# Sue1347/SMSUT-MedicalImgSegmentation

Measured on AMD Instinct MI355X. Metric: slices/sec uganConsisTrainer step @256x256, higher is better.
Workload: dtype f32

## Files before the change

### include/smsut_hip.h

```cpp
#ifndef SMSUT_HIP_H
#define SMSUT_HIP_H

#include <stdint.h>

#ifdef __cplusplus
extern "C" {
#endif

int smsut_conv2d_fwd_generic(const float* x, const float* w, const float* bias , float* y, int N, int H,
                             int W, int Cin, int Ho, int Wo, int Cout, int KH, int KW, int stride, int pad,
                             void* stream);
int smsut_conv2d_dgrad_generic(const float* gy, const float* w, float* gx, int N, int H, int W, int Cin, int Ho, int Wo,
                               int Cout, int KH, int KW, int stride, int pad, void* stream);
int64_t smsut_conv2d_wgrad_generic_ws(int N, int Ho, int Wo, int Cin, int Cout, int KH, int KW);
int smsut_conv2d_wgrad_generic(const float* x, const float* gy, float* gw, float* workspace, int N, int H, int W,
                               int Cin, int Ho, int Wo, int Cout, int KH, int KW, int stride, int pad, void* stream);

int smsut_conv2d_mfma_supported(int KS, int stride, int pad, int Kdim, int Ndim);
int smsut_conv2d_fwd_mfma(const float* x, const float* w, float* y, int N, int H, int W, int Kdim, int Ndim, int KS,
                          int transposed, void* stream);
int smsut_conv2d_mfma_tiles(int N, int H, int W, int Kdim, int Ndim, int KS, int f16);
int smsut_conv2d_mfma_persistent(int N, int H, int W, int Kdim, int Ndim, int KS, int f16);
int smsut_conv2d_dgrad_mfma_bwdstats(const float* gy, const float* w, float* gz, float* stats, const float* y1,
                                     const float* mean, const float* rstd, const float* gamma, const float* beta,
// ... 9 lines not shown
                              int transposed, const float* wu, void* stream);
int smsut_conv2d_fwd_mfma_stats_pre(const float* x, const float* w, float* y, float* stats, int N, int H, int W, int Kdim,
                                    int Ndim, int KS, const float* wu, void* stream);
int smsut_conv2d_dgrad_mfma_bwdstats_pre(const float* gy, const float* w, float* gz, float* stats, const float* y1,
                                         const float* mean, const float* rstd, const float* gamma, const float* beta,
                                         float slope, int N, int H, int W, int Kdim, int Ndim, const float* wu, void* stream);
int smsut_conv2d_fwd_mfma_stats_inaff_pre(const float* x, const float* w, float* y, float* stats, const float* mean,
                                          const float* rstd, const float* gamma, const float* beta, float slope, int N, int H,
                                          int W, int Kdim, int Ndim, const float* wu, void* stream);
int smsut_conv2d_fwd_mfma_stats_cat_pre(const float* xa, const float* xb, const float* w, float* y, float* stats, int N, int H,
                                        int W, int Kdim, int Ndim, const float* wu, void* stream);
int smsut_conv2d_fwd_mfma_split_pre(const float* x, const float* w, float* ya, float* yb, int split, int N, int H, int W,
                                    int Kdim, int Ndim, int transposed, const float* wu, void* stream);
int smsut_conv2d_fwd_mfma_stats_sc_pre(const float* x, const float* xb, const float* w, const float* wsc, float* y, float* ysc,
                                       float* stats, float* stats_sc, int N, int H, int W, int Kdim, int Ndim, const float* wu,
                                       void* stream);
int smsut_conv2d_wgrad_mfma_supported(int KS, int stride, int pad, int Cin, int Cout);
int64_t smsut_conv2d_wgrad_mfma_ws(int N, int H, int W, int Cin, int Cout, int KS);
int smsut_conv2d_wgrad_mfma(const float* x, const float* gy, float* gw, float* workspace, int N, int H, int W, int Cin,
                            int Cout, int KS, void* stream);

int smsut_conv1x1_supported(int Kdim, int Ndim);
int smsut_conv1x1_tiles(int N, int HW, int Ndim);
int smsut_conv1x1_fwd(const float* x, const float* w, float* y, float* stats , int N, int HW, int Kdim,
                      int Ndim, int transposed, void* stream);
int64_t smsut_conv1x1_wgrad_ws(int N, int HW, int Cin, int Cout);
int smsut_conv1x1_wgrad(const float* x, const float* gy, float* gw, float* workspace, int N, int HW, int Cin, int Cout,
                        void* stream);

int smsut_conv2d_fwd_mfma_stats_inaff(const float* x, const float* w, float* y, float* stats, const float* mean,
                                      const float* rstd, const float* gamma, const float* beta, float slope, int N, int H,
                                      int W, int Kdim, int Ndim, void* stream);
int smsut_conv2d_wgrad_mfma_inaff(const float* x, const float* gy, float* gw, float* workspace, const float* mean,
                                  const float* rstd, const float* gamma, const float* beta, float slope, int N, int H, int W,
                                  int Cin, int Cout, void* stream);
int smsut_conv2d_wgrad_mfma_slabs(const float* x, const float* gy, float* workspace, const float* mean, const float* rstd,
                                  const float* gamma, const float* beta, float slope, int N, int H, int W, int Cin, int Cout,
                                  void* stream);
int smsut_conv2d_mfma_form(int N, int H, int W, int Kdim, int Ndim, int sc_dgrad);

int smsut_conv2d_mfma_cat_supported(int N, int H, int W, int Kdim, int Ndim);
int smsut_conv2d_fwd_mfma_stats_cat(const float* xa, const float* xb, const float* w, float* y, float* stats, int N, int H,
                                    int W, int Kdim, int Ndim, void* stream);
int smsut_conv2d_fwd_sc_supported(int N, int H, int W, int Kdim, int Ndim, int cat);
int smsut_conv2d_fwd_mfma_stats_sc(const float* x, const float* xb , const float* w, const float* wsc, float* y,
                                   float* ysc, float* stats, float* stats_sc, int N, int H, int W, int Kdim, int Ndim,
                                   void* stream);
int smsut_conv2d_fwd_sc_f16_supported(int N, int H, int W, int Kdim, int Ndim, int cat);
int smsut_conv2d_fwd_mfma_stats_sc_f16(const float* x, const float* xb, const float* w, const float* wsc, float* y, float* ysc,
                                       float* stats, float* stats_sc, int N, int H, int W, int Kdim, int Ndim, void* stream);
int smsut_conv2d_dgrad_sc_supported(int N, int H, int W, int Cout, int Cin, int split);
int smsut_conv2d_dgrad_mfma_sc(const float* gy, const float* gs, const float* w, const float* wsc, float* gxa,
                               float* gxb , int split, int N, int H, int W, int Cout, int Cin, void* stream);
int smsut_conv2d_wgrad_sc_supported(int N, int H, int W, int Cin, int Cout);
int64_t smsut_conv2d_wgrad_sc_ws(int N, int H, int W, int Cin, int Cout);
int smsut_conv2d_wgrad_mfma_sc(const float* xa, const float* xb , int ca, const float* gy, const float* gs,
                               float* gw10, float* workspace, int N, int H, int W, int Cin, int Cout, void* stream);
int smsut_conv2d_wgrad_mfma_cat(const float* xa, const float* xb, int ca, const float* gy, float* gw, float* workspace,
                                int N, int H, int W, int Cin, int Cout, int KS, void* stream);
int smsut_conv2d_fwd_mfma_stats_sc_fin(const float* x, const float* xb , const float* w, const float* wsc, float* y,
                                       float* ysc, float* stats, float* stats_sc, int* tickets, float* mean, float* rstd,
                                       float* mean_sc, float* rstd_sc, float eps, int N, int H, int W, int Kdim, int Ndim,
                                       const float* wu , void* stream);
int smsut_conv2d_fwd_mfma_stats_inaff_fin(const float* x, const float* w, float* y, float* stats, const float* mean,
                                          const float* rstd, const float* gamma, const float* beta, float slope, int* tickets,
                                          float* mean_out, float* rstd_out, float eps, int N, int H, int W, int Kdim, int Ndim,
                                          const float* wu , void* stream);
int smsut_conv2d_dgrad_mfma_bwdstats_fin(const float* gy, const float* w, float* gz, float* stats, const float* y1,
                                         const float* mean, const float* rstd, const float* gamma, const float* beta, float slope,
                                         int* tickets, float* a_mean, float* b_mean, int N, int H, int W, int Kdim, int Ndim,
                                         const float* wu , void* stream);
int smsut_conv2d_wgrad_pair_supported(int NA, int NB, int H, int W, int Cin, int Cout, int cat, int aff, int sc);
int64_t smsut_conv2d_wgrad_pair_ws(int NA, int NB, int H, int W, int Cin, int Cout, int cat, int aff, int sc);
int smsut_conv2d_wgrad_pair(const float* xA, const float* x2A , const float* gyA, const float* gsA ,
                            const float* meanA , const float* rstdA , int NA, const float* xB,
                            const float* x2B , const float* gyB, const float* gsB ,
                            const float* meanB , const float* rstdB , int NB, int ca,
                            const float* gamma , const float* beta , float slope, float* gw, float* workspace,
                            int H, int W, int Cin, int Cout, void* stream);
int smsut_conv2d_wgrad_pair_slabs(const float* xA, const float* gyA, const float* meanA , const float* rstdA ,
                                  int NA, const float* xB, const float* gyB, const float* meanB ,
                                  const float* rstdB , int NB, const float* gamma , const float* beta ,
                                  float slope, float* workspace, int H, int W, int Cin, int Cout, void* stream);
int smsut_conv1x1_fwd_cat(const float* xa, const float* xb, int ca, const float* w, float* y, float* stats ,
                          int N, int HW, int Kdim, int Ndim, void* stream);
int smsut_conv1x1_wgrad_cat(const float* xa, const float* xb, int ca, const float* gy, float* gw, float* workspace, int N,
                            int HW, int Cin, int Cout, void* stream);

int smsut_conv2d_mfma_split_supported(int N, int H, int W, int Kdim, int Ndim, int split);
int smsut_conv2d_fwd_mfma_split(const float* x, const float* w, float* ya, float* yb, int split, int N, int H, int W,
                                int Kdim, int Ndim, int transposed, void* stream);
int smsut_conv1x1_fwd_split(const float* x, const float* w, float* ya, float* yb, int split, int N, int HW, int Kdim,
                            int Ndim, int transposed, void* stream);

int smsut_conv2d_f16_supported(int KS, int Kdim, int Ndim);
int smsut_conv2d_fwd_mfma_f16(const float* x, const float* w, float* y, const float* gsc , int N, int H, int W,
                              int Kdim, int Ndim, int KS, int transposed, void* stream);
int smsut_conv2d_fwd_mfma_stats_f16(const float* x, const float* w, float* y, float* stats, int N, int H, int W, int Kdim,
                                    int Ndim, int KS, void* stream);
int smsut_conv2d_fwd_mfma_stats_cat_f16(const float* xa, const float* xb, const float* w, float* y, float* stats, int N, int H,
                                        int W, int Kdim, int Ndim, void* stream);
int smsut_conv2d_fwd_mfma_split_f16(const float* x, const float* w, float* ya, float* yb, const float* gsc ,
                                    int split, int N, int H, int W, int Kdim, int Ndim, int transposed, void* stream);
int smsut_conv2d_f16_hs_supported(int N, int H, int W, int Kdim, int Ndim, int cat);
int smsut_conv2d_fwd_mfma_stats_f16_hs(const float* x, const float* xb , const float* w, void* y16, float* stats, int N,
                                       int H, int W, int Kdim, int Ndim, void* stream);
int smsut_conv2d_fwd_mfma_stats_f16_hsx(const void* x16, const float* w, void* y16, float* stats, int N, int H, int W, int Kdim,
                                        int Ndim, void* stream);
int smsut_conv2d_fwd_mfma_stats_inaff_f16_hsx(const void* y1_16, const float* w, void* y16, float* stats, const float* mean,
                                              const float* rstd, const float* gamma, const float* beta, float slope, int N, int H,
                                              int W, int Kdim, int Ndim, void* stream);
int smsut_conv2d_fwd_mfma_stats_sc_f16_hs(const float* x, const float* xb , const float* w, const float* wsc, void* y16,
                                          void* ysc16, float* stats, float* stats_sc, int N, int H, int W, int Kdim, int Ndim,
                                          void* stream);
int smsut_conv2d_dgrad_mfma_bwdstats_f16_hs(const float* gy, const float* w, float* gz, float* stats, const void* y1_16,
                                            const float* mean, const float* rstd, const float* gamma, const float* beta,
                                            const float* gsc , float slope, int N, int H, int W, int Kdim, int Ndim,
                                            void* stream);
int smsut_conv2d_dgrad_sc_f16_supported(int N, int H, int W, int Cout, int Cin, int split);
int smsut_conv2d_dgrad_mfma_sc_f16(const float* gy, const float* gs, const float* w, const float* wsc, float* gxa,
                                   float* gxb , const float* gsc, int split, int N, int H, int W, int Cout, int Cin,
                                   void* stream);
int smsut_conv2d_dgrad_mfma_bwdstats_f16(const float* gy, const float* w, float* gz, float* stats, const float* y1,
                                         const float* mean, const float* rstd, const float* gamma, const float* beta,
                                         const float* gsc , float slope, int N, int H, int W, int Kdim, int Ndim,
                                         void* stream);
int smsut_conv2d_wgrad_f16_supported(int N, int H, int W, int Cin, int Cout);
int64_t smsut_conv2d_wgrad_f16_ws(int N, int H, int W, int Cin, int Cout);
int smsut_conv2d_wgrad_f16(const float* x, const float* x2 , int ca, const float* gy, float* gw, float* workspace,
                           const float* gsc , int N, int H, int W, int Cin, int Cout, void* stream);
int smsut_conv2d_wgrad_f16_xh(const void* x16, const float* gy, float* gw, float* workspace, const float* gsc , int N,
                              int H, int W, int Cin, int Cout, void* stream);
int smsut_conv2d_wgrad_f16_xh_inaff(const void* y1_16, const float* gy, float* gw, float* workspace, const float* gsc ,
                                    const float* mean, const float* rstd, const float* gamma, const float* beta, float slope, int N,
                                    int H, int W, int Cin, int Cout, void* stream);
int smsut_conv2d_wgrad_sc_f16_supported(int N, int H, int W, int Cin, int Cout);
int64_t smsut_conv2d_wgrad_sc_f16_ws(int N, int H, int W, int Cin, int Cout);
int smsut_conv2d_wgrad_sc_f16(const float* x, const float* x2 , int ca, const float* gy, const float* gs, float* gw10,
                              float* workspace, const float* gsc, int N, int H, int W, int Cin, int Cout, void* stream);
int64_t smsut_absmax_scale_ws(int64_t n);
int smsut_absmax_scale(const float* x, int64_t n, float* out2, float* workspace, void* stream);
int smsut_absmax_scale2(const float* x, int64_t n, const float* x2, int64_t n2, float* out2, float* workspace, void* stream);
int smsut_absmax_finish(const float* amax, int n, float* out2, void* stream);

int smsut_conv2d_k4_supported(int Cin, int Cout);
int smsut_conv2d_k4_fwd(const float* x, const float* w, float* y, int N, int H, int W, int Cin, int Cout, int transposed,
                        void* stream);
int64_t smsut_conv2d_k4_wgrad_ws(int N, int H, int W, int Cin, int Cout);
int smsut_conv2d_k4_wgrad(const float* x, const float* gy, float* gw, float* workspace, int N, int H, int W, int Cin, int Cout,
                          void* stream);

int smsut_conv1x1_thin_supported(int Cin, int Cout);
int smsut_conv1x1_thin_dgrad(const float* gy, const float* w, float* gx, int N, int HW, int Cin, int Cout, void* stream);
int64_t smsut_conv1x1_thin_wgrad_ws(int Cin);
int smsut_conv1x1_thin_wgrad(const float* x, const float* gy, float* gw, float* workspace, int N, int HW, int Cin,
                             int Cout, void* stream);

int smsut_conv2d_small_supported(int KS, int Cin, int Cout);
int smsut_conv2d_small_fwd(const float* x, const float* w, const float* bias , float* y, int N, int H, int W,
                           int Cin, int Ho, int Wo, int Cout, int KS, int stride, int pad, void* stream);
int smsut_conv2d_small_dgrad(const float* gy, const float* w, float* gx, int N, int H, int W, int Cin, int Ho, int Wo,
                             int Cout, int KS, int stride, int pad, void* stream);
int smsut_conv2d_flat_wgrad_supported(int KS, int stride, int Cin, int Cout);
int64_t smsut_conv2d_flat_wgrad_ws(int N, int Ho, int Wo, int Cin, int Cout, int KS);
int smsut_conv2d_flat_wgrad(const float* x, const float* gy, float* gw, float* workspace, int N, int H, int W, int Cin,
                            int Ho, int Wo, int Cout, int KS, int stride, int pad, void* stream);
// ... 248 lines not shown
```

### smsut-medicalimgsegmentation_amd/csrc/conv1x1.hip

```cpp
#include "common.h"

namespace {

typedef float f32x4 __attribute__((ext_vector_type(4)));
constexpr int TPB = 256;

__device__ __forceinline__ f32x4 mfma16(float a, float b, f32x4 c) {
  return __builtin_amdgcn_mfma_f32_16x16x4f32(a, b, c, 0, 0, 0);
}

template <int MR, int NR, bool DUAL = false, bool PS = false>
__global__ void __launch_bounds__(TPB)
conv1x1_fwd(const float* __restrict__ x, const float* __restrict__ w, float* __restrict__ y, float* __restrict__ stats,
            int64_t P, int HW, int Kdim, int Ndim, int transposed, float* __restrict__ y2 = nullptr, int split = 0,
            const float* __restrict__ x2 = nullptr, int ca = 0, int ps_w = 0) {
  constexpr int CO_T = 16 * NR;
  extern __shared__ float w_s[];
  const int tid = threadIdx.x, lane = tid & 63, wave = tid >> 6;
  const int lm = lane & 15, kq = lane >> 4;
  const int co0 = blockIdx.y * CO_T;
  const int chunks = (Kdim + 15) / 16;
  for (int u = tid; u < chunks * 4 * CO_T; u += TPB) {
    const int n = u % CO_T;
    const int kg = (u / CO_T) * 4;
    const int ng = co0 + n;
    float4 v = make_float4(0.f, 0.f, 0.f, 0.f);
    if (ng < Ndim && kg < Kdim) {
      if constexpr (PS) {
        const int cout = Ndim >> 2, tap = ng / cout;
        const float* p = w + ((size_t)tap * Kdim + kg) * cout + (ng - tap * cout);
        v.x = p[0]; v.y = p[cout]; v.z = p[2 * (size_t)cout]; v.w = p[3 * (size_t)cout];
      } else if (!transposed) {
        const float* p = w + (size_t)kg * Ndim + ng;
        v.x = p[0]; v.y = p[Ndim]; v.z = p[2 * (size_t)Ndim]; v.w = p[3 * (size_t)Ndim];
      } else {
        v = *(const float4*)(w + (size_t)ng * Kdim + kg);
      }
    }
    *(float4*)(w_s + (size_t)u * 4) = v;
  }
  __syncthreads();

  const int64_t p0 = ((int64_t)blockIdx.x * 4 + wave) * (16 * MR);
  if (p0 >= P) return;
  f32x4 acc[MR][NR];
#pragma unroll
  for (int i = 0; i < MR; ++i)
#pragma unroll
    for (int j = 0; j < NR; ++j) acc[i][j] = (f32x4){0.f, 0.f, 0.f, 0.f};
  const float* xp[MR];
  const float* xq[MR];
  bool pok[MR];
  const int sa = DUAL ? ca : Kdim;
#pragma unroll
  for (int i = 0; i < MR; ++i) {
    const int64_t p = p0 + i * 16 + lm;
    pok[i] = p < P;
    xp[i] = x + (size_t)(pok[i] ? p : 0) * sa + 4 * kq;
    xq[i] = DUAL ? x2 + (size_t)(pok[i] ? p : 0) * (Kdim - ca) + 4 * kq - ca : xp[i];
  }
  for (int c = 0; c < chunks; ++c) {
    const bool kok = c * 16 + 4 * kq < Kdim;
    const bool second = DUAL && c * 16 >= ca;
    f32x4 a[MR], b[NR];
#pragma unroll
    for (int i = 0; i < MR; ++i)
      a[i] = (pok[i] && kok) ? *(const f32x4*)((second ? xq[i] : xp[i]) + c * 16) : (f32x4){0.f, 0.f, 0.f, 0.f};
#pragma unroll
    for (int j = 0; j < NR; ++j) b[j] = *(const f32x4*)(w_s + ((size_t)(c * 4 + kq) * CO_T + j * 16 + lm) * 4);
#pragma unroll
    for (int s = 0; s < 4; ++s)
#pragma unroll
      for (int i = 0; i < MR; ++i)
#pragma unroll
        for (int j = 0; j < NR; ++j) acc[i][j] = mfma16(a[i][s], b[j][s], acc[i][j]);
  }
#pragma unroll
  for (int j = 0; j < NR; ++j) {
    const int co = co0 + j * 16 + lm;
    const bool hi = y2 && co0 + j * 16 >= split;
    float* const yo = hi ? y2 : y;
    const int os = !y2 ? Ndim : (hi ? Ndim - split : split);
    const int oc = hi ? co - split : co;
// ... 56 lines not shown
#pragma unroll
  for (int i = 0; i < CIT; ++i)
#pragma unroll
    for (int j = 0; j < COT; ++j) acc[i][j] = (f32x4){0.f, 0.f, 0.f, 0.f};
  bool iok[CIT], jok[COT];
#pragma unroll
  for (int i = 0; i < CIT; ++i) iok[i] = ci0 + i * 16 + lm < Cin;
#pragma unroll
  for (int j = 0; j < COT; ++j) jok[j] = co0 + j * 16 + lm < Cout;
  CatSrc xs[CIT];
#pragma unroll
  for (int i = 0; i < CIT; ++i) xs[i] = cat_src(x, x2, Cin, ca, ci0 + i * 16);
  const float* gb = gy + co0 + lm;
  [[maybe_unused]] const int cout = Cout >> 2;
  [[maybe_unused]] int ps_tap[COT], ps_cc[COT];
  if constexpr (PS) {
#pragma unroll
    for (int j = 0; j < COT; ++j) { ps_tap[j] = (co0 + j * 16) / cout; ps_cc[j] = co0 + j * 16 - ps_tap[j] * cout + lm; }
  }
  constexpr int UNR = W1_UNR;
  for (int64_t p0 = pb + 4 * wave + kq; p0 - kq < pe; p0 += 16 * UNR) {
    float a[UNR][CIT], b[UNR][COT];
#pragma unroll
    for (int u = 0; u < UNR; ++u) {
      const int64_t p = p0 + 16 * u;
      const bool ok = p < pe;
#pragma unroll
      for (int i = 0; i < CIT; ++i) a[u][i] = (ok && iok[i]) ? xs[i].p[(size_t)p * xs[i].stride + ci0 + i * 16 + lm - xs[i].coff] : 0.f;
      if constexpr (PS) {
        const int row = (int)p / ps_w;
        const int wx = (int)p - row * ps_w;
#pragma unroll
        for (int j = 0; j < COT; ++j)
          b[u][j] = (ok && jok[j]) ? gy[((size_t)(2 * row + (ps_tap[j] >> 1)) * (2 * ps_w) + 2 * wx + (ps_tap[j] & 1)) * cout + ps_cc[j]] : 0.f;
      } else {
#pragma unroll
        for (int j = 0; j < COT; ++j) b[u][j] = (ok && jok[j]) ? gb[(size_t)p * Cout + j * 16] : 0.f;
      }
    }
#pragma unroll
    for (int u = 0; u < UNR; ++u)
#pragma unroll
      for (int i = 0; i < CIT; ++i)
#pragma unroll
        for (int j = 0; j < COT; ++j) acc[i][j] = mfma16(a[u][i], b[u][j], acc[i][j]);
  }
  for (int src = 1; src < 4; ++src) {
    __syncthreads();
    if (wave == src) {
#pragma unroll
      for (int i = 0; i < CIT; ++i)
#pragma unroll
        for (int j = 0; j < COT; ++j) *(f32x4*)(red + ((size_t)(i * COT + j) * 64 + lane) * 4) = acc[i][j];
    }
    __syncthreads();
    if (wave == 0) {
#pragma unroll
      for (int i = 0; i < CIT; ++i)
#pragma unroll
        for (int j = 0; j < COT; ++j) acc[i][j] += *(const f32x4*)(red + ((size_t)(i * COT + j) * 64 + lane) * 4);
    }
  }
  if (wave == 0) {
    float* out = part + (size_t)blockIdx.x * Cin * Cout;
#pragma unroll
    for (int i = 0; i < CIT; ++i)
#pragma unroll
      for (int j = 0; j < COT; ++j) {
        const int co = co0 + j * 16 + lm;
#pragma unroll
        for (int r = 0; r < 4; ++r) {
          const int ci = ci0 + i * 16 + 4 * kq + r;
          if constexpr (PS) {
            if (ci < Cin && co < Cout) out[((size_t)ps_tap[j] * Cin + ci) * cout + ps_cc[j]] = acc[i][j][r];
          } else if (ci < Cin && co < Cout) out[(size_t)ci * Cout + co] = acc[i][j][r];
        }
      }
  }
}

__global__ void __launch_bounds__(TPB)
sum_parts(const float* __restrict__ part, float* __restrict__ out, int wsize, int splits) {
  __shared__ float4 sm[TPB];
  const int col = threadIdx.x & 15, sl = threadIdx.x >> 4;
  const int e = (blockIdx.x * 16 + col) * 4;
  float4 t0 = make_float4(0.f, 0.f, 0.f, 0.f), t1 = t0, t2 = t0, t3 = t0;
  if (e < wsize) {
    int c = sl;
    for (; c + 48 < splits; c += 64) {
      const float4 v0 = *(const float4*)(part + (size_t)c * wsize + e);
      const float4 v1 = *(const float4*)(part + (size_t)(c + 16) * wsize + e);
      const float4 v2 = *(const float4*)(part + (size_t)(c + 32) * wsize + e);
      const float4 v3 = *(const float4*)(part + (size_t)(c + 48) * wsize + e);
      t0.x += v0.x; t0.y += v0.y; t0.z += v0.z; t0.w += v0.w; t1.x += v1.x; t1.y += v1.y; t1.z += v1.z; t1.w += v1.w;
      t2.x += v2.x; t2.y += v2.y; t2.z += v2.z; t2.w += v2.w; t3.x += v3.x; t3.y += v3.y; t3.z += v3.z; t3.w += v3.w;
    }
    for (; c < splits; c += 16) {
      const float4 v = *(const float4*)(part + (size_t)c * wsize + e);
      t0.x += v.x; t0.y += v.y; t0.z += v.z; t0.w += v.w;
    }
  }
  sm[threadIdx.x] = make_float4((t0.x + t1.x) + (t2.x + t3.x), (t0.y + t1.y) + (t2.y + t3.y), (t0.z + t1.z) + (t2.z + t3.z),
                                (t0.w + t1.w) + (t2.w + t3.w));
  __syncthreads();
  if (sl == 0 && e < wsize) {
    float4 t = sm[col];
    for (int l = 1; l < 16; ++l) { const float4 v = sm[l * 16 + col]; t.x += v.x; t.y += v.y; t.z += v.z; t.w += v.w; }
    *(float4*)(out + e) = t;
  }
}

struct Plan1 { int splits; int64_t pps; };
inline Plan1 plan_wgrad1(int64_t P, int Cin, int Cout, int cit, int cot) {
  const int slabs = ((Cin + 16 * cit - 1) / (16 * cit)) * ((Cout + 16 * cot - 1) / (16 * cot));
  int64_t want = (1024 + slabs - 1) / slabs;
  const int64_t maxs = P / 256 > 0 ? P / 256 : 1;
  if (want > maxs) want = maxs;
  if (want < 1) want = 1;
  Plan1 p;
  p.pps = ((P + want - 1) / want + 15) / 16 * 16;
  p.splits = (int)((P + p.pps - 1) / p.pps);
  return p;
}


constexpr int THIN_MAX = 8;

template <int CI>
__global__ void __launch_bounds__(TPB)
thin1x1_dgrad(const float* __restrict__ gy, const float* __restrict__ w, float* __restrict__ gx, int64_t P, int CO) {
  constexpr int Q = CI / 4;
  __shared__ float wt[THIN_MAX * CI];
  for (int u = threadIdx.x; u < THIN_MAX * CI; u += TPB) {
    const int k = u / CI, ci = u % CI;
    wt[u] = k < CO ? w[ci * CO + k] : 0.f;
  }
  __syncthreads();
  const int64_t total = P * Q;
  for (int64_t i = (int64_t)blockIdx.x * TPB + threadIdx.x; i < total; i += (int64_t)gridDim.x * TPB) {
    const int c4 = (int)(i % Q);
    const int64_t px = i / Q;
    float g[THIN_MAX];
#pragma unroll
    for (int k = 0; k < THIN_MAX; ++k) g[k] = k < CO ? gy[px * CO + k] : 0.f;
    f32x4 o = {0.f, 0.f, 0.f, 0.f};
#pragma unroll
    for (int k = 0; k < THIN_MAX; ++k) o += g[k] * *(const f32x4*)(wt + k * CI + c4 * 4);
    *(f32x4*)(gx + i * 4) = o;
  }
}

template <int CI>
__global__ void __launch_bounds__(TPB)
thin1x1_wgrad(const float* __restrict__ x, const float* __restrict__ gy, float* __restrict__ part, int64_t P, int CO) {
  constexpr int Q = CI / 4;
  static_assert(Q <= 64 && (Q & (Q - 1)) == 0, "lanes sharing a channel group sit Q apart inside a wave");
  __shared__ float sm[4 * Q * 4 * THIN_MAX];
  f32x4 acc[THIN_MAX];
#pragma unroll
  for (int k = 0; k < THIN_MAX; ++k) acc[k] = (f32x4){0.f, 0.f, 0.f, 0.f};
  const int64_t total = P * Q;
  const int64_t stride = (int64_t)gridDim.x * TPB;
  auto step = [&](int64_t i) {
    const int64_t px = i / Q;
    const f32x4 xv = *(const f32x4*)(x + i * 4);
#pragma unroll
    for (int k = 0; k < THIN_MAX; ++k) {
      const float g = k < CO ? gy[px * CO + k] : 0.f;
      acc[k] += g * xv;
    }
  };
  int64_t i = (int64_t)blockIdx.x * TPB + threadIdx.x;
  for (; i + stride < total; i += 2 * stride) { step(i); step(i + stride); }
  for (; i < total; i += stride) step(i);
  for (int off = Q; off < 64; off <<= 1) {
#pragma unroll
    for (int k = 0; k < THIN_MAX; ++k)
#pragma unroll
      for (int j = 0; j < 4; ++j) acc[k][j] += __shfl_xor(acc[k][j], off, 64);
  }
  const int lane = threadIdx.x & 63, wv = threadIdx.x >> 6;
  if (lane < Q) {
#pragma unroll
    for (int k = 0; k < THIN_MAX; ++k) *(f32x4*)(sm + ((wv * Q + lane) * THIN_MAX + k) * 4) = acc[k];
  }
  __syncthreads();
  if (threadIdx.x < Q) {
    const int c4 = threadIdx.x;
#pragma unroll
    for (int k = 0; k < THIN_MAX; ++k) {
      f32x4 t = *(const f32x4*)(sm + ((0 * Q + c4) * THIN_MAX + k) * 4);
#pragma unroll
// ... 44 lines not shown
  SMSUT_REQUIRE(!x2 || (!transposed && ca > 0 && ca < Kdim && ca % 16 == 0 && (Kdim - ca) % 4 == 0));
  const int64_t P = (int64_t)N * HW;
  const int mr = (P / 256 >= 512) ? 4 : 1;
  SMSUT_REQUIRE(!stats || HW % (16 * mr) == 0);
  const int nr = Ndim <= 16 ? 1 : 2;
  const int chunks = (Kdim + 15) / 16;
  const size_t sh = (size_t)chunks * 4 * 16 * nr * 4 * sizeof(float);
  dim3 grid((unsigned)cdiv64(P, 64 * mr), (Ndim + 16 * nr - 1) / (16 * nr));
  hipStream_t st = (hipStream_t)stream;
#define LAUNCH1X1(M, R)                                                                                                      \
  do {                                                                                                                       \
    if (x2) conv1x1_fwd<M, R, true><<<grid, TPB, sh, st>>>(x, w, y, stats, P, HW, Kdim, Ndim, transposed, y2, split, x2, ca); \
    else conv1x1_fwd<M, R, false><<<grid, TPB, sh, st>>>(x, w, y, stats, P, HW, Kdim, Ndim, transposed, y2, split, nullptr, 0); \
  } while (0)
  if (mr == 4 && nr == 2) LAUNCH1X1(4, 2);
  else if (mr == 4) LAUNCH1X1(4, 1);
  else if (nr == 2) LAUNCH1X1(1, 2);
  else LAUNCH1X1(1, 1);
#undef LAUNCH1X1
  SMSUT_LAUNCH_CHECK();
  return SMSUT_OK;
}

int smsut_conv1x1_fwd(const float* x, const float* w, float* y, float* stats, int N, int HW, int Kdim, int Ndim,
                      int transposed, void* stream) {
  return conv1x1_fwd_launch(x, w, y, stats, N, HW, Kdim, Ndim, transposed, stream, nullptr, 0);
}

int smsut_conv1x1_fwd_cat(const float* xa, const float* xb, int ca, const float* w, float* y, float* stats, int N, int HW,
                          int Kdim, int Ndim, void* stream) {
  SMSUT_REQUIRE(xb);
  return conv1x1_fwd_launch(xa, w, y, stats, N, HW, Kdim, Ndim, 0, stream, nullptr, 0, xb, ca);
}

int smsut_conv1x1_fwd_split(const float* x, const float* w, float* ya, float* yb, int split, int N, int HW, int Kdim,
                            int Ndim, int transposed, void* stream) {
  SMSUT_REQUIRE(yb);
  return conv1x1_fwd_launch(x, w, ya, nullptr, N, HW, Kdim, Ndim, transposed, stream, yb, split);
}

int smsut_convT2x2_ps_supported(int Cin, int Cout) {
  return Cout == 16 && Cin <= 256 && smsut_conv1x1_supported(Cin, 4 * Cout);
}

int smsut_convT2x2_fwd_ps(const float* x, const float* w, float* y, int N, int H, int W, int Cin, int Cout, void* stream) {
  SMSUT_REQUIRE(x && w && y && N > 0 && H > 0 && W > 0 && smsut_convT2x2_ps_supported(Cin, Cout));
  const int64_t P = (int64_t)N * H * W;
  SMSUT_REQUIRE(P * 4 * Cout < (1ll << 31));
  const int Nd = 4 * Cout;
  const int mr = (P / 256 >= 512) ? 4 : 1;
  const int nr = (Nd % 64 == 0) ? 4 : 2;
  const int chunks = (Cin + 15) / 16;
  const size_t sh = (size_t)chunks * 4 * 16 * nr * 4 * sizeof(float);
  dim3 grid((unsigned)cdiv64(P, 64 * mr), Nd / (16 * nr));
  hipStream_t st = (hipStream_t)stream;
#define PS_GO(M, R) conv1x1_fwd<M, R, false, true><<<grid, TPB, sh, st>>>(x, w, y, nullptr, P, H * W, Cin, Nd, 0, nullptr, 0, nullptr, 0, W)
  if (mr == 4 && nr == 4) PS_GO(4, 4);
  else if (mr == 4) PS_GO(4, 2);
  else if (nr == 4) PS_GO(1, 4);
  else PS_GO(1, 2);
#undef PS_GO
  SMSUT_LAUNCH_CHECK();
  return SMSUT_OK;
}

int64_t smsut_convT2x2_wgrad_ps_ws(int N, int H, int W, int Cin, int Cout) {
  const int cit = Cin > 16 ? 2 : 1;
  return (int64_t)plan_wgrad1((int64_t)N * H * W, Cin, 4 * Cout, cit, 2).splits * Cin * 4 * Cout;
}

int smsut_convT2x2_wgrad_ps(const float* x, const float* gy, float* gw, float* workspace, int N, int H, int W, int Cin,
                            int Cout, void* stream) {
  SMSUT_REQUIRE(x && gy && gw && workspace && N > 0 && H > 0 && W > 0 && smsut_convT2x2_ps_supported(Cin, Cout));
  const int64_t P = (int64_t)N * H * W;
  SMSUT_REQUIRE(P * 4 * Cout < (1ll << 31));
  const int Nd = 4 * Cout;
  const int cit = Cin > 16 ? 2 : 1;
  const Plan1 p = plan_wgrad1(P, Cin, Nd, cit, 2);
  dim3 grid(p.splits, (Cin + 16 * cit - 1) / (16 * cit), Nd / 32);
  hipStream_t st = (hipStream_t)stream;
  if (cit == 2) conv1x1_wgrad<2, 2, true><<<grid, TPB, 0, st>>>(x, gy, workspace, P, Cin, Nd, p.pps, nullptr, 0, W);
  else conv1x1_wgrad<1, 2, true><<<grid, TPB, 0, st>>>(x, gy, workspace, P, Cin, Nd, p.pps, nullptr, 0, W);
  const int wsize = Cin * Nd;
  sum_parts<<<(wsize + 63) / 64, TPB, 0, st>>>(workspace, gw, wsize, p.splits);
  SMSUT_LAUNCH_CHECK();
  return SMSUT_OK;
}

int64_t smsut_conv1x1_wgrad_ws(int N, int HW, int Cin, int Cout) {
  const int cit = Cin > 16 ? 2 : 1, cot = Cout > 16 ? 2 : 1;
  return (int64_t)plan_wgrad1((int64_t)N * HW, Cin, Cout, cit, cot).splits * Cin * Cout;
}

static int conv1x1_wgrad_launch(const float* x, const float* gy, float* gw, float* workspace, int N, int HW, int Cin,
                                int Cout, void* stream, const float* x2, int ca) {
  SMSUT_REQUIRE(x && gy && gw && workspace && N > 0 && HW > 0 && Cin > 0 && Cout > 0);
  SMSUT_REQUIRE(!x2 || (ca > 0 && ca < Cin && ca % 16 == 0));
  SMSUT_REQUIRE(((int64_t)Cin * Cout) % 4 == 0);
  const int64_t P = (int64_t)N * HW;
  const int cit = Cin > 16 ? 2 : 1, cot = Cout > 16 ? 2 : 1;
  const Plan1 p = plan_wgrad1(P, Cin, Cout, cit, cot);
  dim3 grid(p.splits, (Cin + 16 * cit - 1) / (16 * cit), (Cout + 16 * cot - 1) / (16 * cot));
  hipStream_t st = (hipStream_t)stream;
  if (cit == 2 && cot == 2) conv1x1_wgrad<2, 2><<<grid, TPB, 0, st>>>(x, gy, workspace, P, Cin, Cout, p.pps, x2, ca);
  else if (cit == 2) conv1x1_wgrad<2, 1><<<grid, TPB, 0, st>>>(x, gy, workspace, P, Cin, Cout, p.pps, x2, ca);
  else if (cot == 2) conv1x1_wgrad<1, 2><<<grid, TPB, 0, st>>>(x, gy, workspace, P, Cin, Cout, p.pps, x2, ca);
  else conv1x1_wgrad<1, 1><<<grid, TPB, 0, st>>>(x, gy, workspace, P, Cin, Cout, p.pps, x2, ca);
  const int wsize = Cin * Cout;
  sum_parts<<<(wsize + 63) / 64, TPB, 0, st>>>(workspace, gw, wsize, p.splits);
  SMSUT_LAUNCH_CHECK();
  return SMSUT_OK;
}

int smsut_conv1x1_wgrad(const float* x, const float* gy, float* gw, float* workspace, int N, int HW, int Cin, int Cout,
                        void* stream) {
  return conv1x1_wgrad_launch(x, gy, gw, workspace, N, HW, Cin, Cout, stream, nullptr, 0);
}

int smsut_conv1x1_wgrad_cat(const float* xa, const float* xb, int ca, const float* gy, float* gw, float* workspace, int N,
                            int HW, int Cin, int Cout, void* stream) {
  SMSUT_REQUIRE(xb);
  return conv1x1_wgrad_launch(xa, gy, gw, workspace, N, HW, Cin, Cout, stream, xb, ca);
}

int smsut_conv1x1_thin_supported(int Cin, int Cout) {
  return (Cin == 8 || Cin == 16 || Cin == 32 || Cin == 64) && Cout >= 1 && Cout <= THIN_MAX;
}

int smsut_conv1x1_thin_dgrad(const float* gy, const float* w, float* gx, int N, int HW, int Cin, int Cout, void* stream) {
  SMSUT_REQUIRE(gy && w && gx && N > 0 && HW > 0 && smsut_conv1x1_thin_supported(Cin, Cout));
  const int64_t P = (int64_t)N * HW;
  hipStream_t st = (hipStream_t)stream;
  const int grid = ew_grid(P * (Cin / 4));
  switch (Cin) {
    case 8: thin1x1_dgrad<8><<<grid, TPB, 0, st>>>(gy, w, gx, P, Cout); break;
    case 16: thin1x1_dgrad<16><<<grid, TPB, 0, st>>>(gy, w, gx, P, Cout); break;
    case 32: thin1x1_dgrad<32><<<grid, TPB, 0, st>>>(gy, w, gx, P, Cout); break;
    default: thin1x1_dgrad<64><<<grid, TPB, 0, st>>>(gy, w, gx, P, Cout); break;
  }
  SMSUT_LAUNCH_CHECK();
  return SMSUT_OK;
}

int64_t smsut_conv1x1_thin_wgrad_ws(int Cin) { return (int64_t)THIN_WGRAD_BLOCKS * Cin * THIN_MAX; }

int smsut_conv1x1_thin_wgrad(const float* x, const float* gy, float* gw, float* workspace, int N, int HW, int Cin,
                             int Cout, void* stream) {
  SMSUT_REQUIRE(x && gy && gw && workspace && N > 0 && HW > 0 && smsut_conv1x1_thin_supported(Cin, Cout));
  const int64_t P = (int64_t)N * HW;
  hipStream_t st = (hipStream_t)stream;
  int blocks = (int)cdiv64(P * (Cin / 4), 2 * TPB);
  if (blocks > THIN_WGRAD_BLOCKS) blocks = THIN_WGRAD_BLOCKS;
  switch (Cin) {
    case 8: thin1x1_wgrad<8><<<blocks, TPB, 0, st>>>(x, gy, workspace, P, Cout); break;
    case 16: thin1x1_wgrad<16><<<blocks, TPB, 0, st>>>(x, gy, workspace, P, Cout); break;
    case 32: thin1x1_wgrad<32><<<blocks, TPB, 0, st>>>(x, gy, workspace, P, Cout); break;
    default: thin1x1_wgrad<64><<<blocks, TPB, 0, st>>>(x, gy, workspace, P, Cout); break;
  }
  thin1x1_wsum<<<(Cin * THIN_MAX / 4 + 3) / 4, TPB, 0, st>>>(workspace, gw, blocks, Cin, Cout);
  SMSUT_LAUNCH_CHECK();
  return SMSUT_OK;
}

}
```

### smsut-medicalimgsegmentation_amd/csrc/conv_mfma_wgrad.hip

```cpp
#include "conv_mfma.h"
#include "conv_wgrad_rr.h"

namespace {

typedef short s16x4 __attribute__((ext_vector_type(4)));
__device__ __forceinline__ f32x4 mfmak(h4 a, h4 b, f32x4 c) { return mfma16h(a, b, c); }
__device__ __forceinline__ f32x4 mfmak(h8 a, h8 b, f32x4 c) { return mfma32h(a, b, c); }

constexpr int WTH = 8;
#ifndef WG_RR_UNROLL
#define WG_RR_UNROLL 2
#endif
#ifndef WG_KS_UNROLL
#define WG_KS_UNROLL 4
#endif
#ifndef WG11_MIN_BLOCKS
#define WG11_MIN_BLOCKS 1
#endif
#ifndef WTS_STRIDE_VALUE
#define WTS_STRIDE_VALUE 36
#endif
constexpr int WTS_STRIDE_SC = 68;
constexpr int WTS_STRIDE = WTS_STRIDE_VALUE;

template <int KS, int CIT, int COT, bool DUAL = false, bool INAFF = false, bool C8 = false, bool SC8 = false>
__global__ void __launch_bounds__(TPB, (KS == 3 && CIT == 1 && COT == 1 && !INAFF) ? WG11_MIN_BLOCKS : 1)
conv_mfma_wgrad(const float* __restrict__ x, const float* __restrict__ gy, float* __restrict__ part, int N, int H,
                int W, int Cin, int Cout, int tiles_x, int tiles_y, int tiles_per_split, int gsc, int nci,
                const float* __restrict__ x2 = nullptr, int ca = 0, AffRef aff = AffRef{},
                const float* __restrict__ gs = nullptr) {
  static_assert(!SC8 || C8, "fused shortcut weight gradient of the 8-channel form");
  static_assert(!C8 || (KS == 3 && CIT == 1 && !DUAL && !INAFF), "8-channel form: plain 3x3");
  constexpr int KK = KS * KS;
  constexpr int PAD = (KS - 1) / 2;
  constexpr int IH = WTH + KS - 1, IW = TW + KS - 1;
  constexpr int CI_T = 16 * CIT, CO_T = 16 * COT;
  constexpr int SI = (CI_T % 32 == 16) ? CI_T : CI_T + 16;
  constexpr int SO = (CO_T % 32 == 16) ? CO_T : CO_T + 16;
  constexpr int NG = C8 ? (KK + 1) / 2 : KK;
  constexpr int NACC = (NG + (SC8 ? 1 : 0)) * CIT * COT;
  extern __shared__ float smem[];
  float* in_s = smem;
  float* gy_s = smem + IH * IW * SI;
  [[maybe_unused]] float* gs_s = gy_s + WTH * TW * SO;

  const int tid = threadIdx.x;
  const int lane = tid & 63, wave = tid >> 6;
  const int lm = lane & 15, kq = lane >> 4;
  const int split = blockIdx.x;
  const int tg = blockIdx.y / nci;
  const int ci0 = (blockIdx.y % nci) * CI_T, co0 = blockIdx.z * CO_T;
  const int Wg = W * gsc;
  const int tiles_img = tiles_x * tiles_y;
  const int total_tiles = N * tiles_img;
  const int t_begin = split * tiles_per_split;
  const int t_end = min(t_begin + tiles_per_split, total_tiles);

  f32x4 acc[NACC];
#pragma unroll
  for (int i = 0; i < NACC; ++i) acc[i] = (f32x4){0.f, 0.f, 0.f, 0.f};

  constexpr int NIN = (IH * IW * (CI_T / 4) + TPB - 1) / TPB;
  constexpr int NGY = (WTH * TW * (CO_T / 4) + TPB - 1) / TPB;
  float4 rin[NIN], rgy[NGY];
  [[maybe_unused]] float4 rgs[NGY];
  int in_yx[NIN], in_c[NIN], in_lds[NIN], gy_yx[NGY], gy_c[NGY], gy_lds[NGY];
#pragma unroll
  for (int i = 0; i < NIN; ++i) {
    const int u = tid + i * TPB;
    const int q = u % (CI_T / 4), pix = u / (CI_T / 4);
    const int c = ci0 + 4 * q;
    in_yx[i] = (u < IH * IW * (CI_T / 4) && c < Cin) ? (((pix / IW) << 8) | (pix % IW)) : -1;
    in_c[i] = c;
    in_lds[i] = pix * SI + 4 * q;
  }
#pragma unroll
  for (int i = 0; i < NGY; ++i) {
    const int u = tid + i * TPB;
    const int q = u % (CO_T / 4), pix = u / (CO_T / 4);
    const int c = co0 + 4 * q;
    gy_yx[i] = (u < WTH * TW * (CO_T / 4) && c < Cout) ? (((pix / TW) << 8) | (pix % TW)) : -1;
    gy_c[i] = c;
    gy_lds[i] = pix * SO + 4 * q;
  }
// ... 486 lines not shown
        for (int k = 0; k < 9; ++k) {
          const int ti = (wave + 4 * k) >> 1;
          const int tap = ti >> 1, i = ti & 1;
          const auto a = tr_rows(x_h + (i * NPX + (r + tap / KS) * IW + tap % KS) * 16, IW * 16);
          acc[k] = mfmak(a, b, acc[k]);
        }
        if constexpr (SC) {
          const auto bs = tr_rows(s_h + (jt * NPG + r * TW) * 16, TW * 16);
          const auto a = tr_rows(x_h + ((wave >> 1) * NPX + (r + 1) * IW + 1) * 16, IW * 16);
          acc[9] = mfmak(a, bs, acc[9]);
        }
      }
    } else {
#pragma unroll
      for (int rr = 0; rr < WTH / 4; rr += RS) {
        const int r = wave * (WTH / 4) + rr;
        decltype(tr_rows(g_h, 0)) b[COT];
#pragma unroll
        for (int j = 0; j < COT; ++j) b[j] = tr_rows(g_h + (j * NPG + r * TW) * 16, TW * 16);
#pragma unroll
        for (int tap = 0; tap < KK; ++tap)
#pragma unroll
          for (int i = 0; i < CIT; ++i) {
            const auto a = tr_rows(x_h + (i * NPX + (r + tap / KS) * IW + tap % KS) * 16, IW * 16);
#pragma unroll
            for (int j = 0; j < COT; ++j) acc[(tap * CIT + i) * COT + j] = mfmak(a, b[j], acc[(tap * CIT + i) * COT + j]);
          }
        if constexpr (SC) {
          decltype(tr_rows(s_h, 0)) bs[COT];
#pragma unroll
          for (int j = 0; j < COT; ++j) bs[j] = tr_rows(s_h + (j * NPG + r * TW) * 16, TW * 16);
#pragma unroll
          for (int i = 0; i < CIT; ++i) {
            const auto a = tr_rows(x_h + (i * NPX + (r + 1) * IW + 1) * 16, IW * 16);
#pragma unroll
            for (int j = 0; j < COT; ++j) acc[(9 * CIT + i) * COT + j] = mfmak(a, bs[j], acc[(9 * CIT + i) * COT + j]);
          }
        }
      }
    }
  }
  if constexpr (TS) {
    const int jt = wave & 1;
    float* out = part + (size_t)split * KR * Cin * Cout + (size_t)(ci0 + 4 * kq) * Cout + co0 + jt * 16 + lm;
#pragma unroll
    for (int k = 0; k < KR; ++k) {
      const int ti = (wave + 4 * k) >> 1;
      float* o = out + ((ti >> 1) * Cin + (ti & 1) * 16) * Cout;
#pragma unroll
      for (int r = 0; r < 4; ++r) o[r * Cout] = acc[k][r] * gi;
    }
  } else {
    float* red = smem;
    for (int src = 1; src < 4; ++src) {
      __syncthreads();
      if (wave == src) {
#pragma unroll
        for (int k = 0; k < NACC; ++k) *(f32x4*)(red + ((size_t)k * 64 + lane) * 4) = acc[k];
      }
      __syncthreads();
      if (wave == 0) {
#pragma unroll
        for (int k = 0; k < NACC; ++k) acc[k] += *(const f32x4*)(red + ((size_t)k * 64 + lane) * 4);
      }
    }
    if (wave == 0) {
      float* out = part + (size_t)split * KR * Cin * Cout;
#pragma unroll
      for (int tap = 0; tap < KR; ++tap)
#pragma unroll
        for (int i = 0; i < CIT; ++i)
#pragma unroll
          for (int j = 0; j < COT; ++j)
#pragma unroll
            for (int r = 0; r < 4; ++r)
              out[((size_t)tap * Cin + ci0 + i * 16 + 4 * kq + r) * Cout + co0 + j * 16 + lm] = acc[(tap * CIT + i) * COT + j][r] * gi;
    }
  }
}

template <int COLS>
__global__ void __launch_bounds__(TPB)
sum_splits(const float* __restrict__ part, float* __restrict__ out, int wsize, int splits) {
  constexpr int LANES = TPB / COLS;
  __shared__ float4 sm[TPB];
  const int col = threadIdx.x % COLS, sl = threadIdx.x / COLS;
  const int e = (blockIdx.x * COLS + col) * 4;
  float4 t0 = make_float4(0.f, 0.f, 0.f, 0.f), t1 = t0, t2 = t0, t3 = t0;
  if (e < wsize) {
    const float* p = part + e;
    int c = sl;
    for (; c + 3 * LANES < splits; c += 4 * LANES) {
      const float4 v0 = *(const float4*)(p + (size_t)c * wsize);
      const float4 v1 = *(const float4*)(p + (size_t)(c + LANES) * wsize);
      const float4 v2 = *(const float4*)(p + (size_t)(c + 2 * LANES) * wsize);
      const float4 v3 = *(const float4*)(p + (size_t)(c + 3 * LANES) * wsize);
      t0.x += v0.x; t0.y += v0.y; t0.z += v0.z; t0.w += v0.w;
      t1.x += v1.x; t1.y += v1.y; t1.z += v1.z; t1.w += v1.w;
      t2.x += v2.x; t2.y += v2.y; t2.z += v2.z; t2.w += v2.w;
      t3.x += v3.x; t3.y += v3.y; t3.z += v3.z; t3.w += v3.w;
    }
    for (; c < splits; c += LANES) {
      const float4 v = *(const float4*)(p + (size_t)c * wsize);
      t0.x += v.x; t0.y += v.y; t0.z += v.z; t0.w += v.w;
    }
  }
  sm[threadIdx.x] = make_float4((t0.x + t1.x) + (t2.x + t3.x), (t0.y + t1.y) + (t2.y + t3.y),
                                (t0.z + t1.z) + (t2.z + t3.z), (t0.w + t1.w) + (t2.w + t3.w));
  __syncthreads();
  if (sl == 0 && e < wsize) {
    float4 t = sm[col];
    for (int l = 1; l < LANES; ++l) {
      const float4 v = sm[l * COLS + col];
      t.x += v.x; t.y += v.y; t.z += v.z; t.w += v.w;
    }
    *(float4*)(out + e) = t;
  }
}

inline void launch_sum_splits(const float* part, float* out, int wsize, int splits, hipStream_t st) {
  if (wsize >= 32768) sum_splits<64><<<(wsize + 255) / 256, TPB, 0, st>>>(part, out, wsize, splits);
  else if (wsize >= 8192) sum_splits<32><<<(wsize + 127) / 128, TPB, 0, st>>>(part, out, wsize, splits);
  else sum_splits<16><<<(wsize + 63) / 64, TPB, 0, st>>>(part, out, wsize, splits);
}

constexpr int PW_UNR = 8;
__global__ void __launch_bounds__(TPB)
plane_wgrad(const float* __restrict__ x, const float* __restrict__ gy, float* __restrict__ gw, int N, int H, int W, int Cin,
            int Cout, const float* __restrict__ x2 = nullptr, int ca = 0) {
  __shared__ float red[3 * 4 * 64 * 4];
  const int lane = threadIdx.x & 63, wave = threadIdx.x >> 6;
  const int lm = lane & 15, kq = lane >> 4;
  const int ci0 = blockIdx.x * 32, co0 = blockIdx.y * 32;
  const int tap = blockIdx.z, dy = tap / 3 - 1, dx = tap % 3 - 1;
  const int HW = H * W, P = N * HW;
  f32x4 acc[2][2];
#pragma unroll
  for (int i = 0; i < 2; ++i)
#pragma unroll
    for (int j = 0; j < 2; ++j) acc[i][j] = (f32x4){0.f, 0.f, 0.f, 0.f};
  const CatSrc s0 = cat_src(x, x2, Cin, ca, ci0), s1 = cat_src(x, x2, Cin, ca, ci0 + 16);
  const float* xa0 = s0.p + ci0 + lm - s0.coff;
  const float* xa1 = s1.p + ci0 + 16 + lm - s1.coff;
  const float* gb = gy + co0 + lm;
  constexpr int BLK = 4 * PW_UNR;
  for (int p0 = wave * BLK; p0 < P; p0 += 4 * BLK) {
    const int pk = p0 + kq;
    int cn = pk / HW;
    const int r = pk - cn * HW;
    int cy = r / W, cx = r - cy * W;
    float a[PW_UNR][2], b[PW_UNR][2];
#pragma unroll
    for (int u = 0; u < PW_UNR; ++u) {
      const int p = p0 + 4 * u + kq;
      const int yy = cy + dy, xx = cx + dx;
      const bool ok = p < P;
      const bool in = ok && yy >= 0 && yy < H && xx >= 0 && xx < W;
      const size_t pix = (size_t)((cn * H + yy) * W + xx);
      const float* gp = gb + (size_t)p * Cout;
      a[u][0] = in ? xa0[pix * s0.stride] : 0.f; a[u][1] = in ? xa1[pix * s1.stride] : 0.f;
      b[u][0] = ok ? gp[0] : 0.f; b[u][1] = ok ? gp[16] : 0.f;
      cx += 4;
      if (cx >= W) { cx -= W; if (++cy == H) { cy = 0; ++cn; } }
    }
#pragma unroll
    for (int u = 0; u < PW_UNR; ++u)
#pragma unroll
      for (int i = 0; i < 2; ++i)
#pragma unroll
        for (int j = 0; j < 2; ++j) acc[i][j] = mfma16(a[u][i], b[u][j], acc[i][j]);
  }
  if (wave > 0) {
#pragma unroll
    for (int t = 0; t < 4; ++t) *(f32x4*)(red + (((wave - 1) * 4 + t) * 64 + lane) * 4) = acc[t >> 1][t & 1];
  }
  __syncthreads();
  if (wave == 0) {
#pragma unroll
    for (int t = 0; t < 4; ++t) {
      f32x4 v = acc[t >> 1][t & 1];
#pragma unroll
      for (int w4 = 0; w4 < 3; ++w4) v += *(const f32x4*)(red + ((w4 * 4 + t) * 64 + lane) * 4);
      float* o = gw + ((size_t)tap * Cin + ci0 + (t >> 1) * 16 + 4 * kq) * Cout + co0 + (t & 1) * 16 + lm;
#pragma unroll
      for (int r = 0; r < 4; ++r) o[(size_t)r * Cout] = v[r];
    }
  }
}

template <int COT>
__global__ void __launch_bounds__(TPB)
conv_k4_wgrad(const float* __restrict__ x, const float* __restrict__ gy, float* __restrict__ part, int N, int Hi, int Wi,
              int Ho, int Wo, int Cin, int Cout, int tiles_x, int tiles_y, int tiles_per_split) {
  constexpr int KS = 4, KK = 16, PAD = 1;
  constexpr int IH = WTH + KS - 1, IW = TW + KS - 1;
  constexpr int CO_T = 16 * COT, SI = 16, SO = (CO_T % 32 == 16) ? CO_T : CO_T + 16;
  constexpr int NACC = KK * COT;
  extern __shared__ float smem[];
  float* in_s = smem;
  float* gy_s = smem + IH * IW * SI;
  const int tid = threadIdx.x, lane = tid & 63, wave = tid >> 6;
  const int lm = lane & 15, kq = lane >> 4;
  const int split = blockIdx.x, ci0 = blockIdx.y * 16, co0 = blockIdx.z * CO_T;
  const int tiles_img = tiles_x * tiles_y, total_tiles = N * tiles_img;
  const int t_begin = split * tiles_per_split, t_end = min(t_begin + tiles_per_split, total_tiles);
  f32x4 acc[NACC];
#pragma unroll
// ... 226 lines not shown
  }
  if (c.aff) return c.x2 ? -1 : go(conv_mfma_wgrad_ts<false, true>, sh);
  return c.x2 ? go(conv_mfma_wgrad_ts<true>, sh) : go(conv_mfma_wgrad_ts<false>, sh);
}

inline WgradCall wgrad_call(const void* x, const float* x2, int ca, const float* gy, float* part, int N, int H, int W, int Cin, int Cout,
                            void* stream) {
  WgradCall c;
  c.x = x; c.x2 = x2; c.ca = x2 ? ca : 0; c.gy = gy; c.part = part;
  c.N = N; c.H = H; c.W = W; c.Cin = Cin; c.Cout = Cout; c.stream = (hipStream_t)stream;
  return c;
}
inline int wgrad_reduce(int rc, const WgradCall& c, const WgradPlan& p, float* gw) {
  SMSUT_REQUIRE(rc == 0);
  launch_sum_splits(c.part, gw, p.rows * c.Cin * c.Cout, p.splits, c.stream);
  SMSUT_LAUNCH_CHECK();
  return SMSUT_OK;
}

int wgrad_run(const WgradCall& c, float* gw) {
  SMSUT_REQUIRE(c.x && c.gy && c.part && c.N > 0 && c.H > 0 && c.W > 0);
  SMSUT_REQUIRE(!c.x2 || (c.ca > 0 && c.ca < c.Cin && c.ca % 16 == 0 && (c.Cin - c.ca) % 4 == 0));
  const WgradKey k = c.key();
  WgradPlan p = wgrad_select(k, c.KS);
  if (p.fam == WF_RR && smsut_wgrad_rr_launch(c) != 0) p = wgrad_select(k, c.KS, true);
  if (c.b || !gw) SMSUT_REQUIRE(p.fam == WF_RR);
  if (!gw) return hipGetLastError() == hipSuccess ? p.splits : SMSUT_EINVAL;
  switch (p.fam) {
    case WF_NONE: return SMSUT_EINVAL;
    case WF_RR: return wgrad_reduce(0, c, p, gw);
    case WF_TS: return wgrad_reduce(launch_wgrad_ts(c, p), c, p, gw);
    case WF_PLANE:
      plane_wgrad<<<dim3(c.Cin / 32, c.Cout / 32, 9), TPB, 0, c.stream>>>((const float*)c.x, c.gy, gw, c.N, c.H, c.W, c.Cin, c.Cout,
                                                                        c.x2, c.ca);
      SMSUT_LAUNCH_CHECK();
      return SMSUT_OK;
    default: return wgrad_reduce(launch_wgrad_rows(c, p), c, p, gw);
  }
}

inline bool wgrad_f16_shape_ok(int N, int H, int W, int Cin, int Cout) {
  return N > 0 && H > 0 && W > 0 && H % WTH == 0 && W % TW == 0 && Cin % 16 == 0 && Cout % 16 == 0 &&
         (int64_t)N * H * W * (Cin > Cout ? Cin : Cout) < (1ll << 31);
}
WgradPlan plan_wgrad_f16(int N, int H, int W, int Cin, int Cout, bool sc) {
  WgradPlan p = plan_wgrad(N, H, W, Cin, Cout);
  p.cit = (Cin % 32 == 0) ? 2 : 1;
  p.cot = (Cout % 32 == 0) ? 2 : 1;
  p.rows = sc ? 10 : 9;
  return p;
}
template <int CI, int CO>
int launch_wgrad_f16(const WgradCall& c, const WgradPlan& p) {
  constexpr int NPX = (WTH + 2) * (TW + 2), NPG = WTH * TW;
  const bool sc = c.gs != nullptr;
  const size_t stage = (size_t)((CI * NPX + (sc ? 2 : 1) * CO * NPG) * 16 + 8) * sizeof(_Float16);
  const size_t red = (CI == 2 && CO == 2) ? 0 : (size_t)p.rows * CI * CO * 64 * 4 * sizeof(float);
  const dim3 grid(p.splits, c.Cin / (16 * CI), c.Cout / (16 * CO));
  auto go = [&](auto kern) {
    kern<<<grid, TPB, stage > red ? stage : red, c.stream>>>((const float*)c.x, c.gy, c.part, c.N, c.H, c.W, c.Cin, c.Cout, p.tiles_x,
                                                             p.tiles_y, p.tiles_per_split, c.x2, c.ca, c.gsc, c.gs,
                                                             c.aff ? *c.aff : AffRef{});
    return 0;
  };
  if (c.x_f16) {
    if (c.x2 || sc) return -1;
    return c.aff ? go(conv_f16_wgrad<CI, CO, false, false, true, true>) : go(conv_f16_wgrad<CI, CO, false, false, true>);
  }
  if (c.aff) return -1;
  if (sc) return c.x2 ? go(conv_f16_wgrad<CI, CO, true, true>) : go(conv_f16_wgrad<CI, CO, false, true>);
  return c.x2 ? go(conv_f16_wgrad<CI, CO, true, false>) : go(conv_f16_wgrad<CI, CO, false, false>);
}
int wgrad_f16_run(const WgradCall& c, float* gw) {
  SMSUT_REQUIRE(c.x && c.gy && gw && c.part && wgrad_f16_shape_ok(c.N, c.H, c.W, c.Cin, c.Cout));
  SMSUT_REQUIRE(!c.x2 || (c.ca > 0 && c.ca < c.Cin && c.ca % 16 == 0));
  const WgradPlan p = plan_wgrad_f16(c.N, c.H, c.W, c.Cin, c.Cout, c.gs != nullptr);
  const int rc = p.cit == 2 ? (p.cot == 2 ? launch_wgrad_f16<2, 2>(c, p) : launch_wgrad_f16<2, 1>(c, p))
                            : (p.cot == 2 ? launch_wgrad_f16<1, 2>(c, p) : launch_wgrad_f16<1, 1>(c, p));
  return wgrad_reduce(rc, c, p, gw);
}

}

extern "C" {

#ifdef SMSUT_STAMPS
int smsut_dbg_wgrad_stamps(void* buf, int base) {
  (void)hipMemcpyToSymbol(HIP_SYMBOL(g_stamp_base), &base, sizeof(base));
  return (int)hipMemcpyToSymbol(HIP_SYMBOL(g_stamps), &buf, sizeof(buf));
}
#endif
#ifdef SMSUT_DBG_SUM
int smsut_dbg_sum_splits(const float* part, float* out, int wsize, int splits, void* stream) {
  launch_sum_splits(part, out, wsize, splits, (hipStream_t)stream);
  return 0;
}
#endif

int smsut_conv2d_wgrad_mfma_supported(int KS, int stride, int pad, int Cin, int Cout) {
  return (KS == 1 || KS == 3) && stride == 1 && pad == (KS - 1) / 2 && wgrad_channels_ok(Cin, Cout);
}

int64_t smsut_conv2d_wgrad_mfma_ws(int N, int H, int W, int Cin, int Cout, int KS) {
  return wgrad_ws_floats(WgradKey{N, H, W, Cin, Cout, false, false, false}, KS);
}

int smsut_conv2d_wgrad_mfma(const float* x, const float* gy, float* gw, float* workspace, int N, int H, int W, int Cin,
                            int Cout, int KS, void* stream) {
  SMSUT_REQUIRE(gw);
  WgradCall c = wgrad_call(x, nullptr, 0, gy, workspace, N, H, W, Cin, Cout, stream);
  c.KS = KS;
  return wgrad_run(c, gw);
}

int smsut_conv2d_wgrad_mfma_inaff(const float* x, const float* gy, float* gw, float* workspace, const float* mean,
                                  const float* rstd, const float* gamma, const float* beta, float slope, int N, int H, int W,
                                  int Cin, int Cout, void* stream) {
  SMSUT_REQUIRE(gw && mean && rstd && gamma && beta);
  const AffRef a{mean, rstd, gamma, beta, slope};
  WgradCall c = wgrad_call(x, nullptr, 0, gy, workspace, N, H, W, Cin, Cout, stream);
  c.aff = &a;
  return wgrad_run(c, gw);
}

int smsut_conv2d_wgrad_mfma_slabs(const float* x, const float* gy, float* workspace, const float* mean, const float* rstd,
                                  const float* gamma, const float* beta, float slope, int N, int H, int W, int Cin, int Cout,
                                  void* stream) {
  SMSUT_REQUIRE(!mean || (rstd && gamma && beta));
  const AffRef a{mean, rstd, gamma, beta, slope};
  WgradCall c = wgrad_call(x, nullptr, 0, gy, workspace, N, H, W, Cin, Cout, stream);
  c.aff = mean ? &a : nullptr;
  return wgrad_run(c, nullptr);
}

int smsut_conv2d_wgrad_sc_supported(int N, int H, int W, int Cin, int Cout) {
  return wgrad_select(WgradKey{N, H, W, Cin, Cout, false, false, true}, 3).fam != WF_NONE;
}
int64_t smsut_conv2d_wgrad_sc_ws(int N, int H, int W, int Cin, int Cout) {
  return wgrad_ws_floats(WgradKey{N, H, W, Cin, Cout, false, false, true}, 3);
}
int smsut_conv2d_wgrad_mfma_sc(const float* xa, const float* xb, int ca, const float* gy, const float* gs, float* gw10,
                               float* workspace, int N, int H, int W, int Cin, int Cout, void* stream) {
  SMSUT_REQUIRE(gw10 && gs);
  WgradCall c = wgrad_call(xa, xb, ca, gy, workspace, N, H, W, Cin, Cout, stream);
  c.gs = gs;
  return wgrad_run(c, gw10);
}

int smsut_conv2d_wgrad_mfma_cat(const float* xa, const float* xb, int ca, const float* gy, float* gw, float* workspace,
                                int N, int H, int W, int Cin, int Cout, int KS, void* stream) {
  SMSUT_REQUIRE(gw && xb);
  WgradCall c = wgrad_call(xa, xb, ca, gy, workspace, N, H, W, Cin, Cout, stream);
  c.KS = KS;
  return wgrad_run(c, gw);
}

int smsut_conv2d_wgrad_pair_supported(int NA, int NB, int H, int W, int Cin, int Cout, int cat, int aff, int sc) {
  return NA > 0 && NB > 0 && wgrad_select(WgradKey{NA + NB, H, W, Cin, Cout, cat != 0, aff != 0, sc != 0}, 3).fam == WF_RR;
}
int64_t smsut_conv2d_wgrad_pair_ws(int NA, int NB, int H, int W, int Cin, int Cout, int cat, int aff, int sc) {
  return (int64_t)smsut_wgrad_rr_splits(WgradKey{NA + NB, H, W, Cin, Cout, cat != 0, aff != 0, sc != 0}) * (sc ? 10 : 9) * Cin * Cout;
}
static int wgrad_pair_run(const WgradSetB& sa, const WgradSetB& sb, int ca, const float* gamma, const float* beta, float slope, float* gw,
                          float* workspace, int H, int W, int Cin, int Cout, void* stream) {
  const bool aff = sa.mean != nullptr;
  SMSUT_REQUIRE(aff == (sa.rstd != nullptr) && (!aff || (gamma && beta)));
  const AffRef a{sa.mean, sa.rstd, gamma, beta, slope};
// ... 118 lines not shown
```

### smsut-medicalimgsegmentation_amd/csrc/conv_naive.hip

```cpp
#include "common.h"

namespace {

constexpr int TPB = 256;

struct ConvGeom {
  int N, H, W, Cin, Ho, Wo, Cout, KH, KW, stride, pad;
};

__global__ void __launch_bounds__(TPB)
conv_fwd_naive(const float* __restrict__ x, const float* __restrict__ w, const float* __restrict__ bias,
               float* __restrict__ y, ConvGeom g, int64_t total) {
  for (int64_t i = (int64_t)blockIdx.x * TPB + threadIdx.x; i < total; i += (int64_t)gridDim.x * TPB) {
    const int co = (int)(i % g.Cout);
    int64_t p = i / g.Cout;
    const int wo = (int)(p % g.Wo); p /= g.Wo;
    const int ho = (int)(p % g.Ho);
    const int n = (int)(p / g.Ho);
    float acc = bias ? bias[co] : 0.f;
    for (int kh = 0; kh < g.KH; ++kh) {
      const int hi = ho * g.stride - g.pad + kh;
      if (hi < 0 || hi >= g.H) continue;
      for (int kw = 0; kw < g.KW; ++kw) {
        const int wi = wo * g.stride - g.pad + kw;
        if (wi < 0 || wi >= g.W) continue;
        const float* xp = x + (((size_t)n * g.H + hi) * g.W + wi) * g.Cin;
        const float* wp = w + ((size_t)(kh * g.KW + kw) * g.Cin) * g.Cout + co;
        for (int ci = 0; ci < g.Cin; ++ci) acc = fmaf(xp[ci], wp[(size_t)ci * g.Cout], acc);
      }
    }
    y[i] = acc;
  }
}

__global__ void __launch_bounds__(TPB)
conv_full_window(const float* __restrict__ x, const float* __restrict__ w, const float* __restrict__ bias,
                 float* __restrict__ y, int K, int Cout) {
  __shared__ float sm4[4];
  const int n = blockIdx.x;
  for (int co = 0; co < Cout; ++co) {
    float acc = 0.f;
    for (int k = threadIdx.x; k < K; k += TPB) acc = fmaf(x[(size_t)n * K + k], w[(size_t)k * Cout + co], acc);
    const float t = block_sum_256(acc, sm4);
    if (threadIdx.x == 0) y[(size_t)n * Cout + co] = t + (bias ? bias[co] : 0.f);
  }
}

__global__ void __launch_bounds__(TPB)
conv_dgrad_naive(const float* __restrict__ gy, const float* __restrict__ w, float* __restrict__ gx, ConvGeom g,
                 int64_t total) {
  for (int64_t i = (int64_t)blockIdx.x * TPB + threadIdx.x; i < total; i += (int64_t)gridDim.x * TPB) {
    const int ci = (int)(i % g.Cin);
    int64_t p = i / g.Cin;
    const int wi = (int)(p % g.W); p /= g.W;
    const int hi = (int)(p % g.H);
    const int n = (int)(p / g.H);
    float acc = 0.f;
    for (int kh = 0; kh < g.KH; ++kh) {
      const int hn = hi + g.pad - kh;
      if (hn < 0 || hn % g.stride) continue;
      const int ho = hn / g.stride;
      if (ho >= g.Ho) continue;
      for (int kw = 0; kw < g.KW; ++kw) {
        const int wn = wi + g.pad - kw;
        if (wn < 0 || wn % g.stride) continue;
        const int wo = wn / g.stride;
        if (wo >= g.Wo) continue;
        const float* gp = gy + (((size_t)n * g.Ho + ho) * g.Wo + wo) * g.Cout;
        const float* wp = w + ((size_t)(kh * g.KW + kw) * g.Cin + ci) * g.Cout;
        int co = 0;
        if ((g.Cout & 3) == 0) {
          for (; co < g.Cout; co += 4) {
            const float4 a = *(const float4*)(gp + co);
            const float4 b = *(const float4*)(wp + co);
            acc = fmaf(a.x, b.x, acc); acc = fmaf(a.y, b.y, acc);
            acc = fmaf(a.z, b.z, acc); acc = fmaf(a.w, b.w, acc);
          }
        } else {
          for (; co < g.Cout; ++co) acc = fmaf(gp[co], wp[co], acc);
        }
      }
    }
    gx[i] = acc;
  }
}

__global__ void __launch_bounds__(TPB)
conv_wgrad_partial(const float* __restrict__ x, const float* __restrict__ gy, float* __restrict__ part, ConvGeom g,
                   int wsize, int64_t npix, int pix_per_chunk) {
  const int e = blockIdx.x * TPB + threadIdx.x;
  const int chunk = blockIdx.y;
  if (e >= wsize) return;
  const int co = e % g.Cout;
  int t = e / g.Cout;
  const int ci = t % g.Cin; t /= g.Cin;
  const int kw = t % g.KW;
  const int kh = t / g.KW;
  const int64_t p0 = (int64_t)chunk * pix_per_chunk;
  const int64_t p1 = min(p0 + (int64_t)pix_per_chunk, npix);
  int wo = (int)(p0 % g.Wo);
  const int64_t q0 = p0 / g.Wo;
  int ho = (int)(q0 % g.Ho);
  int n = (int)(q0 / g.Ho);
  float acc = 0.f;
  const float* gp = gy + (size_t)p0 * g.Cout + co;
  for (int64_t p = p0; p < p1; ++p, gp += g.Cout) {
    const int hi = ho * g.stride - g.pad + kh;
    const int wi = wo * g.stride - g.pad + kw;
    if (hi >= 0 && hi < g.H && wi >= 0 && wi < g.W)
      acc = fmaf(x[(((size_t)n * g.H + hi) * g.W + wi) * g.Cin + ci], *gp, acc);
    if (++wo == g.Wo) { wo = 0; if (++ho == g.Ho) { ho = 0; ++n; } }
  }
  part[(size_t)chunk * wsize + e] = acc;
}

__global__ void __launch_bounds__(TPB)
reduce_chunks(const float* __restrict__ part, float* __restrict__ out, int wsize, int chunks) {
  __shared__ double sm[TPB];
  const int e = blockIdx.x * 64 + (threadIdx.x & 63);
  const int lane_c = threadIdx.x >> 6;
  double s = 0.0;
  if (e < wsize) {
    int c = lane_c;
    for (; c + 28 < chunks; c += 32) {
      float v[8];
#pragma unroll
      for (int u = 0; u < 8; ++u) v[u] = part[(size_t)(c + 4 * u) * wsize + e];
#pragma unroll
      for (int u = 0; u < 8; ++u) s += (double)v[u];
    }
    for (; c < chunks; c += 4) s += (double)part[(size_t)c * wsize + e];
  }
  sm[threadIdx.x] = s;
  __syncthreads();
  if (lane_c == 0 && e < wsize)
    out[e] = (float)(sm[threadIdx.x] + sm[threadIdx.x + 64] + sm[threadIdx.x + 128] + sm[threadIdx.x + 192]);
}

__global__ void __launch_bounds__(TPB)
colsum_partial(const float* __restrict__ x, float* __restrict__ part, int64_t rows, int C, int rows_per_chunk) {
  const int chunk = blockIdx.x;
  const int64_t r0 = (int64_t)chunk * rows_per_chunk;
  const int64_t r1 = min(r0 + (int64_t)rows_per_chunk, rows);
  const int TC = C < TPB ? C : TPB;
  const int nrow = TPB / TC;
  const int tc = threadIdx.x % TC, tr = threadIdx.x / TC;
  __shared__ float sm[TPB];
  for (int c0 = 0; c0 < C; c0 += TC) {
    const int c = c0 + tc;
    float acc = 0.f;
    if (tr < nrow && c < C) {
      int64_t r = r0 + tr;
      for (; r + 7 * (int64_t)nrow < r1; r += 8 * (int64_t)nrow) {
        float v[8];
#pragma unroll
        for (int u = 0; u < 8; ++u) v[u] = x[(size_t)(r + u * (int64_t)nrow) * C + c];
#pragma unroll
        for (int u = 0; u < 8; ++u) acc += v[u];
      }
      for (; r < r1; r += nrow) acc += x[(size_t)r * C + c];
    }
    __syncthreads();
    sm[threadIdx.x] = acc;
    __syncthreads();
    if (tr == 0 && c < C) {
      float tot = 0.f;
      for (int r = 0; r < nrow; ++r) tot += sm[r * TC + tc];
      part[(size_t)chunk * C + c] = tot;
    }
    __syncthreads();
  }
}

inline int wgrad_ppc(int64_t npix, int wsize) {
  const int64_t chunks_target = wsize <= 4096 ? 8192 : 1024;
  int64_t ppc = cdiv64(npix, chunks_target);
  if (ppc < 64) ppc = 64;
  return (int)ppc;
}

inline bool geom_ok(const ConvGeom& g) {
  if (g.N <= 0 || g.H <= 0 || g.W <= 0 || g.Cin <= 0 || g.Cout <= 0 || g.KH <= 0 || g.KW <= 0 || g.stride <= 0 ||
      g.pad < 0)
    return false;
  return g.Ho == (g.H + 2 * g.pad - g.KH) / g.stride + 1 && g.Wo == (g.W + 2 * g.pad - g.KW) / g.stride + 1 &&
         g.Ho > 0 && g.Wo > 0;
}

}

extern "C" {

int smsut_conv2d_fwd_generic(const float* x, const float* w, const float* bias, float* y, int N, int H, int W, int Cin,
                             int Ho, int Wo, int Cout, int KH, int KW, int stride, int pad, void* stream) {
  ConvGeom g{N, H, W, Cin, Ho, Wo, Cout, KH, KW, stride, pad};
  SMSUT_REQUIRE(x && w && y && geom_ok(g));
  const int64_t total = (int64_t)N * Ho * Wo * Cout;
  if (KH == H && KW == W && pad == 0 && Cout <= 16)
    conv_full_window<<<N, TPB, 0, (hipStream_t)stream>>>(x, w, bias, y, KH * KW * Cin, Cout);
  else
    conv_fwd_naive<<<ew_grid(total) * 4, TPB, 0, (hipStream_t)stream>>>(x, w, bias, y, g, total);
  SMSUT_LAUNCH_CHECK();
  return SMSUT_OK;
}

int smsut_conv2d_dgrad_generic(const float* gy, const float* w, float* gx, int N, int H, int W, int Cin, int Ho, int Wo,
                               int Cout, int KH, int KW, int stride, int pad, void* stream) {
  ConvGeom g{N, H, W, Cin, Ho, Wo, Cout, KH, KW, stride, pad};
  SMSUT_REQUIRE(gy && w && gx && geom_ok(g));
  const int64_t total = (int64_t)N * H * W * Cin;
  conv_dgrad_naive<<<ew_grid(total) * 4, TPB, 0, (hipStream_t)stream>>>(gy, w, gx, g, total);
  SMSUT_LAUNCH_CHECK();
  return SMSUT_OK;
}

int64_t smsut_conv2d_wgrad_generic_ws(int N, int Ho, int Wo, int Cin, int Cout, int KH, int KW) {
  const int64_t npix = (int64_t)N * Ho * Wo;
  const int ppc = wgrad_ppc(npix, KH * KW * Cin * Cout);
  return cdiv64(npix, ppc) * (int64_t)KH * KW * Cin * Cout;
}

int smsut_conv2d_wgrad_generic(const float* x, const float* gy, float* gw, float* workspace, int N, int H, int W,
                               int Cin, int Ho, int Wo, int Cout, int KH, int KW, int stride, int pad, void* stream) {
  ConvGeom g{N, H, W, Cin, Ho, Wo, Cout, KH, KW, stride, pad};
  SMSUT_REQUIRE(x && gy && gw && workspace && geom_ok(g));
  const int64_t npix = (int64_t)N * Ho * Wo;
  const int wsize = KH * KW * Cin * Cout;
  const int ppc = wgrad_ppc(npix, wsize);
  const int chunks = (int)cdiv64(npix, ppc);
  hipStream_t st = (hipStream_t)stream;
  conv_wgrad_partial<<<dim3((wsize + TPB - 1) / TPB, chunks), TPB, 0, st>>>(x, gy, workspace, g, wsize, npix, ppc);
  reduce_chunks<<<(wsize + 63) / 64, TPB, 0, st>>>(workspace, gw, wsize, chunks);
  SMSUT_LAUNCH_CHECK();
  return SMSUT_OK;
}

int64_t smsut_colsum_ws(int64_t rows, int C) {
  int64_t rpc = cdiv64(rows, 512);
  if (rpc < 64) rpc = 64;
  return cdiv64(rows, rpc) * C;
}

int smsut_colsum(const float* x, float* out, float* workspace, int64_t rows, int C, void* stream) {
  SMSUT_REQUIRE(x && out && workspace && rows > 0 && C > 0);
  int64_t rpc = cdiv64(rows, 512);
  if (rpc < 64) rpc = 64;
  const int chunks = (int)cdiv64(rows, rpc);
  hipStream_t st = (hipStream_t)stream;
  colsum_partial<<<chunks, TPB, 0, st>>>(x, workspace, rows, C, (int)rpc);
  reduce_chunks<<<(C + 63) / 64, TPB, 0, st>>>(workspace, out, C, chunks);
  SMSUT_LAUNCH_CHECK();
  return SMSUT_OK;
}

}
```

### smsut-medicalimgsegmentation_amd/ops.py

```python
from __future__ import annotations

import contextlib
import math
import os as _os
from typing import NamedTuple, Optional

import torch
from torch.autograd import Function
from torch.autograd.function import once_differentiable

from . import _hip as H

IN_EPS = 1e-5

_INPUT_GRADS_ONLY = False


@contextlib.contextmanager
def input_grads_only():
    global _INPUT_GRADS_ONLY
    prev, _INPUT_GRADS_ONLY = _INPUT_GRADS_ONLY, True
    try:
        yield
    finally:
# ... 716 lines not shown

def res_tail_pool(y2, g2, b2, s, gs, bs, slope):
    return ResTailFn.apply(y2, g2, b2, s, gs, bs, slope, True)


FUSED_BLOCK = bool(int(_os.environ.get("SMSUT_FUSED_BLOCK", "1")))
FUSED_RES_TAIL = bool(int(_os.environ.get("SMSUT_FUSED_RES_TAIL", "1")))
VIRTUAL_CAT = bool(int(_os.environ.get("SMSUT_VIRTUAL_CAT", "1")))
SPLIT_DGRAD = bool(int(_os.environ.get("SMSUT_SPLIT_DGRAD", "1")))
AMAX_HANDOVER = bool(int(_os.environ.get("SMSUT_AMAX_HANDOVER", "1")))


def basic_block_fusable(x, w1, ws):
    co, ci = w1.shape[0], w1.shape[1]
    return (FUSED_BLOCK and x.is_cuda and ci % 4 == 0 and co % 4 == 0 and ci >= 4 and co >= 4
            and (ws is not None or ci == co))


FIN_ON = bool(int(_os.environ.get("SMSUT_FIN", "1")))
_TICKET_RING = {}
_TICKET_CHUNKS = {}
_TICKET_KEEP = []
_TICKET_RING_INTS = 1 << 20
_TICKET_CHUNK_INTS = 1 << 13


def _tickets(n: int, like: torch.Tensor):
    if not FIN_ON:
        return None
    from . import graphs
    dev = like.device.index or 0
    if graphs._CAPTURING > 0:
        key = (dev, graphs.CAPTURE_SEQ)
        ent = _TICKET_CHUNKS.get(key)
        if ent is None or ent[1] + n > ent[0].numel():
            ent = _TICKET_CHUNKS[key] = [torch.zeros(max(_TICKET_CHUNK_INTS, n), dtype=torch.int32, device=like.device), 0]
            _TICKET_KEEP.append(ent[0])
        t = ent[0][ent[1]:ent[1] + n]
        ent[1] += n
        return t
    if torch.cuda.is_current_stream_capturing():
        return None
    ent = _TICKET_RING.get(dev)
    if ent is None:
        ent = _TICKET_RING[dev] = [torch.zeros(_TICKET_RING_INTS, dtype=torch.int32, device=like.device), 0]
    if ent[1] + n > _TICKET_RING_INTS:
        ent[1] = 0
    t = ent[0][ent[1]:ent[1] + n]
    ent[1] += n
    return t


def _fin_available(like: torch.Tensor) -> bool:
    return _tickets(0, like) is not None


def _wu(w, transposed):
    return _WINO_ACTIVE.get((w.data_ptr(), transposed & 1)) if _WINO_ACTIVE else None


_PAIR_FWD = False
_PAIR_STASH = {}


@contextlib.contextmanager
def pair_wgrads():
    global _PAIR_FWD
    prev, _PAIR_FWD = _PAIR_FWD, True
    try:
        yield
    finally:
        _PAIR_FWD = prev


def pair_reset():
    _PAIR_STASH.clear()


def pair_flush():
    if not _PAIR_STASH:
        return 0
    n = 0
    for key in list(_PAIR_STASH):
        for mine, single, deliver in _PAIR_STASH.pop(key):
            deliver(single(mine))
            n += 1
    return n


def pair_assert_empty():
    if _PAIR_STASH:
        n = sum(len(v) for v in _PAIR_STASH.values())
        _PAIR_STASH.clear()
        raise RuntimeError(f"ops.pair_wgrads: {n} parked weight-gradient operand set(s) were never computed (pair_flush() missing "
                           "at the end of the iteration's last backward)")


def _add_grad(p, g):
    if p.grad is None:
        p.grad = g
    else:
        p.grad = p.grad + g


class WgradSet(NamedTuple):
    x: torch.Tensor; x2: Optional[torch.Tensor]; gy: torch.Tensor; gs: Optional[torch.Tensor]
    mean: Optional[torch.Tensor]; rstd: Optional[torch.Tensor]; n: int


def _pair_wgrad(key, mine: WgradSet, launch, single, deliver):
    rows, ca, gamma, beta, slope, dims = launch
    lst = _PAIR_STASH.get(key)
    if not lst:
        _PAIR_STASH.setdefault(key, []).append((mine, single, deliver))
        return None
    other = lst.pop()[0]
    if not lst:
        del _PAIR_STASH[key]
    cat, aff, sc = int(mine.x2 is not None), int(mine.mean is not None), int(mine.gs is not None)
    if not H.call("smsut_conv2d_wgrad_pair_supported", mine.n, other.n, *dims, cat, aff, sc):
        return single(mine) + single(other)
    gw = torch.empty(rows * dims[2] * dims[3], dtype=torch.float32, device=mine.x.device)
    ws = _ws(H.call("smsut_conv2d_wgrad_pair_ws", mine.n, other.n, *dims, cat, aff, sc), mine.x)
    H.call("smsut_conv2d_wgrad_pair", *mine, *other, ca, gamma if aff else None, beta if aff else None, float(slope), gw, ws, *dims, _s())
    return gw


class BlockPlan(NamedTuple):
    n: int; h: int; w: int; ci: int; co: int
    cat: Optional[tuple]; has_sc: bool; virtual: bool; pool: bool; slope: float
    f16a: bool; f16: bool; hs: bool; fused_sc: bool; fin: bool; inaff: bool; pair: bool
    t3: int; t3b: int


def _block_plan(like, cat, virtual, co, has_sc, slope, pool) -> BlockPlan:
    n, ci, h, w = like.shape
    ci, vc = (cat[0] + cat[1], 1) if virtual else (ci, 0)
    f16a = CONV_F16 and ci % 16 == 0 and co % 16 == 0
    f16 = CONV_F16 and co % 16 == 0
    t3 = H.call("smsut_conv2d_mfma_tiles", n, h, w, ci, co, 3, int(f16a))
    t3b = H.call("smsut_conv2d_mfma_tiles", n, h, w, co, co, 3, int(f16))
    fused_sc = has_sc and bool(H.call("smsut_conv2d_fwd_sc_f16_supported" if f16a else "smsut_conv2d_fwd_sc_supported", n, h, w, ci, co, vc))
    hs = ((f16a or ci == 8) and f16 and fused_sc and bool(H.call("smsut_conv2d_f16_hs_supported", n, h, w, ci, co, vc))
          and bool(H.call("smsut_conv2d_f16_hs_supported", n, h, w, co, co, 0)))
    inaff = not f16 and co % 16 == 0 and bool(H.call("smsut_conv2d_mfma_persistent", n, h, w, co, co, 3, 0))
    fin = fused_sc and not (f16a or hs) and inaff and _fin_available(like)
    return BlockPlan(n, h, w, ci, co, cat, has_sc, virtual, pool, slope, f16a, f16, hs, fused_sc, fin, inaff, _PAIR_FWD and not CONV_F16, t3, t3b)


def _bb_conv1(p: BlockPlan, x, x2, w1, ws, st):
    n, h, w, ci, co = p[:5]
    act_dt = torch.float16 if p.hs else torch.float32
    s = ps = ms = rs = None
    p1 = _ws(n * p.t3 * co * 2, x)
    y1 = new_act(n, co, h, w, x, act_dt)
    if p.fused_sc:
        s, ps = new_act(n, co, h, w, x, act_dt), _ws(n * p.t3 * co * 2, x)
    m1, r1 = _vec(x, n, co), _vec(x, n, co)
    if p.hs:
        H.call("smsut_conv2d_fwd_mfma_stats_sc_f16_hs", x, x2, w1, ws, y1, s, p1, ps, n, h, w, ci, co, st)
    elif p.fin:
        ms, rs = _vec(x, n, co), _vec(x, n, co)
        H.call("smsut_conv2d_fwd_mfma_stats_sc_fin", x, x2, w1, ws, y1, s, p1, ps, _tickets(n, x), m1, r1, ms, rs, IN_EPS,
               n, h, w, ci, co, _wu(w1, 0), st)
    elif p.fused_sc:
        _conv3("smsut_conv2d_fwd_mfma_stats_sc_f16" if p.f16a else "smsut_conv2d_fwd_mfma_stats_sc", w1, 0, x, x2, w1, ws, y1, s,
               p1, ps, n, h, w, ci, co, st)
    elif p.virtual:
        _conv3("smsut_conv2d_fwd_mfma_stats_cat_f16" if p.f16a else "smsut_conv2d_fwd_mfma_stats_cat", w1, 0, x, x2, w1, y1, p1, n, h, w, ci, co, st)
    else:
        _conv3("smsut_conv2d_fwd_mfma_stats_f16" if p.f16a else "smsut_conv2d_fwd_mfma_stats", w1, 0, x, w1, y1, p1, n, h, w, ci, co, 3, st)
    return y1, p1, m1, r1, s, ps, ms, rs


def _bb_conv2(p: BlockPlan, y1, p1, m1, r1, g1, b1, w2, ps, ms, rs, st):
    n, h, w, _, co = p[:5]
    hw, slope, a1 = h * w, p.slope, None
    y2 = new_act(n, co, h, w, y1, torch.float16 if p.hs else torch.float32)
    p2 = _ws(n * p.t3b * co * 2, y1)
    if p.fin:
        m2, r2 = _vec(y1, n, co), _vec(y1, n, co)
        H.call("smsut_conv2d_fwd_mfma_stats_inaff_fin", y1, w2, y2, p2, m1, r1, g1, b1, slope, _tickets(n, y1), m2, r2, IN_EPS,
               n, h, w, co, co, _wu(w2, 0), st)
    elif p.inaff:
        H.call("smsut_in_finalize_fwd", p1, p.t3, m1, r1, n, hw, co, IN_EPS, st)
        _conv3("smsut_conv2d_fwd_mfma_stats_inaff", w2, 0, y1, w2, y2, p2, m1, r1, g1, b1, slope, n, h, w, co, co, st)
    elif p.hs:
        H.call("smsut_in_finalize_fwd", p1, p.t3, m1, r1, n, hw, co, IN_EPS, st)
        H.call("smsut_conv2d_fwd_mfma_stats_inaff_f16_hsx", y1, w2, y2, p2, m1, r1, g1, b1, slope, n, h, w, co, co, st)
    else:
        a1 = new_act(n, co, h, w, y1)
        H.call("smsut_instnorm_fwd_partials", y1, g1, b1, a1, m1, r1, p1, p.t3, n, hw, co, IN_EPS, slope, 1, st)
        _conv3("smsut_conv2d_fwd_mfma_stats_f16" if p.f16 else "smsut_conv2d_fwd_mfma_stats", w2, 0, a1, w2, y2, p2, n, h, w, co, co, 3, st)
    if not p.fin:
        m2, r2 = _vec(y1, n, co), _vec(y1, n, co)
        if p.fused_sc:
            ms, rs = _vec(y1, n, co), _vec(y1, n, co)
            H.call("smsut_in_finalize_fwd2", p2, p.t3b, m2, r2, ps, p.t3, ms, rs, n, hw, co, IN_EPS, st)
        else:
            H.call("smsut_in_finalize_fwd", p2, p.t3b, m2, r2, n, hw, co, IN_EPS, st)
    return y2, a1, m2, r2, ms, rs


def _bb_shortcut(p: BlockPlan, x, x2, ws, st):
    n, h, w, ci, co = p[:5]
    hw, s = h * w, new_act(n, co, h, w, x)
    t1s = H.call("smsut_conv1x1_tiles", n, hw, co) if H.call("smsut_conv1x1_supported", ci, co) else 0
    t1 = t1s if (t1s or p.virtual) else H.call("smsut_conv2d_mfma_tiles", n, h, w, ci, co, 1, 0)
# ... 40 lines not shown
    chunks = H.call("smsut_in_chunks", n, h * w, co)
    nb = H.call("smsut_amax_blocks", n, h * w, co) if (f16 or f16a) and AMAX_HANDOVER else 0
    fin_ok = not hs and not nb and (mp or has_sc) and fin_available()
    tail = "pool" if mp else "hs" if hs else "amax" if nb else "fin" if fin_ok else "plain"
    pers2 = bool(H.call("smsut_conv2d_mfma_persistent", n, h, w, co, co, 3, int(f16)))
    fin_b = pers2 and p.fin and fin_ok
    amax1 = pers2 and nb > 0 and (hs or f16a)
    f16w2 = f16 and bool(H.call("smsut_conv2d_wgrad_f16_supported", n, h, w, co, co))
    f16w1 = f16a and bool(H.call("smsut_conv2d_wgrad_f16_supported", n, h, w, ci, co))
    pair2 = p.pair and bool(H.call("smsut_conv2d_wgrad_pair_supported", n, n, h, w, co, co, 0, int(p.inaff), 0))
    split_c = p.cat[0] if cat else 0
    fused_wsc16 = has_sc and f16w1 and bool(H.call("smsut_conv2d_wgrad_sc_f16_supported", n, h, w, ci, co))
    fused_dsc16 = (has_sc and f16a and (needs[0] or needs[11] or needs[12])
                   and bool(H.call("smsut_conv2d_dgrad_sc_f16_supported", n, h, w, co, ci, split_c)))
    fused_wsc = fused_wsc16 or (has_sc and not f16w1 and bool(H.call("smsut_conv2d_wgrad_sc_supported", n, h, w, ci, co)))
    pair1 = p.pair and fused_wsc and bool(H.call("smsut_conv2d_wgrad_pair_supported", n, n, h, w, ci, co, int(p.virtual), 0, 1))
    dx = None
    if (needs[11] or needs[12]) if cat else needs[0]:
        if fused_dsc16:
            dx = "sc_f16"
        elif has_sc and not f16a and H.call("smsut_conv2d_dgrad_sc_supported", n, h, w, co, ci, split_c):
            dx = "sc"
        elif (cat and has_sc and split_c % 16 == 0 and H.call("smsut_conv1x1_supported", co, ci)
                and H.call("smsut_conv2d_mfma_split_supported", n, h, w, co, ci, split_c)):
            dx = "split"
        else:
            dx = "accum" if not has_sc or H.call("smsut_conv1x1_supported", co, ci) else "accum_k1"
    return BlockBwd(chunks, nb, amax1, tail, fin_ok, pers2, fin_b, f16w1, f16w2, pair1, pair2, fused_wsc16, fused_wsc, fused_dsc16, dx)


def _bb_tail_bwd(p: BlockPlan, b: BlockBwd, g_out, g_pooled, pool_idx, out, y2, m2, r2, g2, b2, s, ms, rs, gs, bs, st):
    n, h, w, _, co = p[:5]
    hw, slope = h * w, p.slope
    gy2, gs_t = new_act(n, co, h, w, y2), new_act(n, co, h, w, y2)
    a_t, b2_t, bs_t = _vec(y2, n, co), _vec(y2, n, co), _vec(y2, n, co)
    gg2, gb2 = _vec(y2, co), _vec(y2, co)
    ggs, gbs = (_vec(y2, co), _vec(y2, co)) if p.has_sc else (None, None)
    amax = _vec(y2, 3 * b.nb) if b.nb else None
    tk = _tickets(n, y2) if b.tail == "pool" and b.fin_ok else None
    io = (y2, m2, r2, g2, b2, s, ms, rs, gs, bs, gy2, gs_t, a_t, b2_t, bs_t, gg2, gb2, ggs, gbs, _ws(n * b.chunks * co * 3, y2))
    if b.tail == "pool":
        H.call("smsut_restail_bwd_pool", g_out, g_pooled, pool_idx, *io, tk, amax, n, h, w, co, slope, int(p.hs), st)
    elif b.tail in ("hs", "amax"):
        H.call("smsut_restail_bwd_hs" if p.hs else "smsut_restail_bwd_amax", g_out, out, *io, amax, n, hw, co, slope, st)
    elif b.tail == "fin":
        H.call("smsut_restail_bwd_fin", g_out, out, *io, _tickets(n, y2), n, hw, co, slope, st)
    else:
        H.call("smsut_restail_bwd", g_out, out, *io, n, hw, co, slope, st)
    return gy2, gs_t, gg2, gb2, ggs, gbs, amax


def _bb_dgrad2(p: BlockPlan, b: BlockBwd, gy2, w2, y1, m1, r1, g1, b1, amax, st):
    n, h, w, _, co = p[:5]
    hw, slope, f16, hs, nb = h * w, p.slope, p.f16, p.hs, b.nb
    ga1, gy1 = new_act(n, co, h, w, gy2), new_act(n, co, h, w, gy2)
    a1m, b1m, gg1, gb1 = _vec(gy2, n, co), _vec(gy2, n, co), _vec(gy2, co), _vec(gy2, co)
    sc2 = (_grad_scale_from(amax[:nb]) if amax is not None else _grad_scale(gy2)) if f16 else None
    if not b.pers2:
        if f16:
            H.call("smsut_conv2d_fwd_mfma_f16", gy2, w2, ga1, sc2, n, h, w, co, co, 3, 1, st)
        else:
            _conv3("smsut_conv2d_fwd_mfma", w2, 1, gy2, w2, ga1, n, h, w, co, co, 3, 1, st)
        H.call("smsut_instnorm_bwd", ga1, y1, b1, m1, r1, g1, gy1, a1m, b1m, gg1, gb1, _ws(n * b.chunks * co * 3, gy2), n, hw, co, slope, st)
        return gy1, gg1, gb1, sc2
    pb = _ws(n * p.t3b * co * 2, gy2)
    if f16:
        H.call("smsut_conv2d_dgrad_mfma_bwdstats_f16_hs" if hs else "smsut_conv2d_dgrad_mfma_bwdstats_f16", gy2, w2, ga1, pb, y1, m1, r1, g1, b1,
               sc2, slope, n, h, w, co, co, st)
    elif b.fin_b:
        H.call("smsut_conv2d_dgrad_mfma_bwdstats_fin", gy2, w2, ga1, pb, y1, m1, r1, g1, b1, slope, _tickets(n, gy2), a1m, b1m,
               n, h, w, co, co, _wu(w2, 1), st)
    else:
        _conv3("smsut_conv2d_dgrad_mfma_bwdstats", w2, 1, gy2, w2, ga1, pb, y1, m1, r1, g1, b1, slope, n, h, w, co, co, st)
    if not b.fin_b:
        H.call("smsut_in_finalize_bwd", pb, p.t3b, a1m, b1m, n, hw, co, st)
    if hs or b.amax1:
        H.call("smsut_in_apply_bwd_hs" if hs else "smsut_in_apply_bwd_amax", ga1, y1, m1, r1, g1, a1m, b1m, gy1, gg1, gb1,
               amax[2 * nb:] if b.amax1 else None, n, hw, co, st)
    else:
        H.call("smsut_in_apply_bwd", ga1, y1, m1, r1, g1, a1m, b1m, gy1, gg1, gb1, n, hw, co, st)
    return gy1, gg1, gb1, sc2


def _bb_wgrad2(p: BlockPlan, b: BlockBwd, pair_w, y1, a1, gy2, w2, sc2, m1, r1, g1, b1, st):
    (n, h, w, _, co), slope = p[:5], p.slope
    if p.hs or b.f16w2:
        gw2 = new_weight(co, co, 3, 3, device=gy2.device)
        wws = _ws(H.call("smsut_conv2d_wgrad_f16_ws", n, h, w, co, co), gy2)
        if p.hs:
            H.call("smsut_conv2d_wgrad_f16_xh_inaff", y1, gy2, gw2, wws, sc2, m1, r1, g1, b1, slope, n, h, w, co, co, st)
        else:
            H.call("smsut_conv2d_wgrad_f16", a1, None, 0, gy2, gw2, wws, sc2, n, h, w, co, co, st)
        return gw2

    def single2(t):
        g = _vec(t.x, 9 * co * co)
        wws2 = _ws(H.call("smsut_conv2d_wgrad_mfma_ws", t.n, h, w, co, co, 3), t.x)
        if t.mean is not None:
            H.call("smsut_conv2d_wgrad_mfma_inaff", t.x, t.gy, g, wws2, t.mean, t.rstd, g1, b1, slope, t.n, h, w, co, co, _s())
        else:
            H.call("smsut_conv2d_wgrad_mfma", t.x, t.gy, g, wws2, t.n, h, w, co, co, 3, _s())
        return g
    as_w2 = lambda g: torch.as_strided(g, (co, co, 3, 3), hwio_strides(co, co, 3, 3))
    mine2 = WgradSet(y1, None, gy2, None, m1, r1, n) if p.inaff else WgradSet(a1, None, gy2, None, None, None, n)
    if not b.pair2:
        return as_w2(single2(mine2))
    leaf2 = pair_w[1]
    gw2 = _pair_wgrad(("w2", w2.data_ptr()), mine2, (9, 0, g1, b1, slope, (h, w, co, co)), single2, lambda g: _add_grad(leaf2, as_w2(g)))
    return None if gw2 is None else as_w2(gw2)


def _bb_wgrad1(p: BlockPlan, b: BlockBwd, pair_w, x, x2, gy1, gs_t, w1, amax, st):
    n, h, w, ci, co = p[:5]
    hw, ca = h * w, (p.cat[0] if p.virtual else 0)
    as_w1 = lambda g: torch.as_strided(g, (co, ci, 3, 3), hwio_strides(co, ci, 3, 3))
    as_ws = lambda g: torch.as_strided(g, (co, ci, 1, 1), hwio_strides(co, ci, 1, 1), 9 * ci * co)
    if not p.f16a:
        sc1 = None
    elif b.fused_wsc16 or b.fused_dsc16:
        sc1 = _grad_scale_from(amax[b.nb:]) if b.amax1 else _grad_scale2(gy1, gs_t)
    else:
        sc1 = _grad_scale_from(amax[2 * b.nb:]) if b.amax1 else _grad_scale(gy1)
    if b.fused_wsc16:
        g10 = _vec(x, 10 * ci * co)
        H.call("smsut_conv2d_wgrad_sc_f16", x, x2, ca, gy1, gs_t, g10, _ws(H.call("smsut_conv2d_wgrad_sc_f16_ws", n, h, w, ci, co), x),
               sc1, n, h, w, ci, co, st)
        return as_w1(g10), as_ws(g10), sc1
    if b.fused_wsc:
        def single1(t):
            g = _vec(t.x, 10 * ci * co)
            H.call("smsut_conv2d_wgrad_mfma_sc", t.x, t.x2, ca, t.gy, t.gs, g,
                   _ws(H.call("smsut_conv2d_wgrad_sc_ws", t.n, h, w, ci, co), t.x), t.n, h, w, ci, co, _s())
            return g
        mine1 = WgradSet(x, x2, gy1, gs_t, None, None, n)
        if b.pair1:
            leaf1, leafs = pair_w[0], pair_w[2]
            g10 = _pair_wgrad(("w1", w1.data_ptr()), mine1, (10, ca, None, None, p.slope, (h, w, ci, co)), single1,
                              lambda g: (_add_grad(leaf1, as_w1(g)), _add_grad(leafs, as_ws(g))))
        else:
            g10 = single1(mine1)
        return (None, None, sc1) if g10 is None else (as_w1(g10), as_ws(g10), sc1)
    gw1 = new_weight(co, ci, 3, 3, device=x.device)
    wws = _ws(H.call("smsut_conv2d_wgrad_f16_ws", n, h, w, ci, co) if b.f16w1 else H.call("smsut_conv2d_wgrad_mfma_ws", n, h, w, ci, co, 3), x)
    if b.f16w1:
        H.call("smsut_conv2d_wgrad_f16", x, x2, ca, gy1, gw1, wws, sc1, n, h, w, ci, co, st)
    elif p.virtual:
        H.call("smsut_conv2d_wgrad_mfma_cat", x, x2, ca, gy1, gw1, wws, n, h, w, ci, co, 3, st)
    else:
        H.call("smsut_conv2d_wgrad_mfma", x, gy1, gw1, wws, n, h, w, ci, co, 3, st)
    if not p.has_sc:
        return gw1, None, sc1
    gws = new_weight(co, ci, 1, 1, device=x.device)
    wws1 = _ws(H.call("smsut_conv1x1_wgrad_ws", n, hw, ci, co), x)
    if p.virtual:
        H.call("smsut_conv1x1_wgrad_cat", x, x2, ca, gs_t, gws, wws1, n, hw, ci, co, st)
    else:
        H.call("smsut_conv1x1_wgrad", x, gs_t, gws, wws1, n, hw, ci, co, st)
    return gw1, gws, sc1


def _bb_dgrad1(p: BlockPlan, b: BlockBwd, gy1, gs_t, w1, ws, sc1, st):
    n, h, w, ci, co = p[:5]
    hw, split = h * w, p.cat is not None
    ca, cb = p.cat if split else (0, 0)
    ga, gb = (new_act(n, ca, h, w, gy1), new_act(n, cb, h, w, gy1)) if split else (None, None)
    gx = None if (split and b.dx[:5] != "accum") else new_act(n, ci, h, w, gy1) if p.has_sc else gs_t
    d0, d1 = (ga, gb) if split else (gx, None)
    if b.dx == "sc_f16":
        H.call("smsut_conv2d_dgrad_mfma_sc_f16", gy1, gs_t, w1, ws, d0, d1, sc1, ca, n, h, w, co, ci, st)
    elif b.dx == "sc":
        H.call("smsut_conv2d_dgrad_mfma_sc", gy1, gs_t, w1, ws, d0, d1, ca, n, h, w, co, ci, st)
    elif b.dx == "split":
        H.call("smsut_conv1x1_fwd_split", gs_t, ws, ga, gb, ca, n, hw, co, ci, 1, st)
        if p.f16a:
            H.call("smsut_conv2d_fwd_mfma_split_f16", gy1, w1, ga, gb, sc1, ca, n, h, w, co, ci, 3, st)
        else:
            _conv3("smsut_conv2d_fwd_mfma_split", w1, 1, gy1, w1, ga, gb, ca, n, h, w, co, ci, 3, st)
    else:
        if b.dx == "accum_k1":
            H.call("smsut_conv2d_fwd_mfma", gs_t, ws, gx, n, h, w, co, ci, 1, 1, st)
        elif p.has_sc:
            H.call("smsut_conv1x1_fwd", gs_t, ws, gx, None, n, hw, co, ci, 1, st)
        if p.f16a:
            H.call("smsut_conv2d_fwd_mfma_f16", gy1, w1, gx, sc1, n, h, w, co, ci, 3, 3, st)
        else:
            _conv3("smsut_conv2d_fwd_mfma", w1, 1, gy1, w1, gx, n, h, w, co, ci, 3, 3, st)
        if split:
            H.call("smsut_concat2", ga, ca, gb, cb, gx, n * hw, 1, st)
    return (None, ga, gb) if split else (gx, None, None)


class BasicBlockFn(Function):

    @staticmethod
    def forward(ctx, x, w1, g1, b1, w2, g2, b2, ws, gs, bs, slope, xa=None, xb=None, pool=False):
        leaves = (w1, w2, ws)
        cat = (xa.shape[1], xb.shape[1]) if xa is not None else None
        x, x2 = (nhwc(xa), nhwc(xb)) if x is None else (nhwc(x), None)
        w1, w2, ws = hwio(w1), hwio(w2), (hwio(ws) if ws is not None else None)
        p = ctx.plan = _block_plan(x, cat, x2 is not None, w1.shape[0], ws is not None, float(slope), bool(pool))
        st = _s()
        y1, p1, m1, r1, s, ps, ms, rs = _bb_conv1(p, x, x2, w1, ws, st)
        y2, a1, m2, r2, ms, rs = _bb_conv2(p, y1, p1, m1, r1, g1, b1, w2, ps, ms, rs, st)
        if p.has_sc and not p.fused_sc:
            s, ms, rs = _bb_shortcut(p, x, x2, ws, st)
        out, pooled, ctx.pool_idx = _bb_tail(p, y2, m2, r2, g2, b2, s if p.has_sc else x, ms, rs, gs, bs, st)
        ctx.pair_w = leaves if p.pair else None
        ctx.set_materialize_grads(False)
        ctx.save_for_backward(x, x2, w1, w2, ws, y1, a1, y2, s, out, m1, r1, m2, r2, ms, rs, g1, b1, g2,
                              *((gs, b2, bs) if p.has_sc else (None, None, None)))
        return (out, pooled) if pool else out

    @staticmethod
    @once_differentiable
    def backward(ctx, g_out, g_pooled=None):
        p = ctx.plan
        x, x2, w1, w2, ws, y1, a1, y2, s, out, m1, r1, m2, r2, ms, rs, g1, b1, g2, gs, b2, bs = ctx.saved_tensors
        if p.pool and g_out is None:
            g_out = new_act(p.n, p.co, p.h, p.w, x)
            H.call("smsut_maxpool2_bwd", nhwc(g_pooled), out, g_out, p.n, p.h, p.w, p.co, _s())
            g_pooled = None
        g_out = nhwc(g_out)
        mp = p.pool and g_pooled is not None
        g_pooled = nhwc(g_pooled) if mp else None
        b = _block_bwd_plan(p, ctx.needs_input_grad, mp, lambda: _fin_available(x))
        st = _s()
        gy2, gs_t, gg2, gb2, ggs, gbs, amax = _bb_tail_bwd(p, b, g_out, g_pooled, ctx.pool_idx, out, y2, m2, r2, g2, b2,
                                                           s if p.has_sc else x, ms, rs, gs, bs, st)
        gy1, gg1, gb1, sc2 = _bb_dgrad2(p, b, gy2, w2, y1, m1, r1, g1, b1, amax, st)
        gw2 = _bb_wgrad2(p, b, ctx.pair_w, y1, a1, gy2, w2, sc2, m1, r1, g1, b1, st)
        gw1, gws, sc1 = _bb_wgrad1(p, b, ctx.pair_w, x, x2, gy1, gs_t, w1, amax, st)
        gx, ga, gb = _bb_dgrad1(p, b, gy1, gs_t, w1, ws, sc1, st) if b.dx else (None, None, None)
        return gx, gw1, gg1, gb1, gw2, gg2, gb2, gws, ggs, gbs, None, ga, gb, None


class CatParts:
    __slots__ = ("a", "b", "_t")

    def __init__(self, a, b):
        self.a, self.b, self._t = a, b, None

    @property
    def shape(self):
        return torch.Size((self.a.shape[0], self.a.shape[1] + self.b.shape[1], self.a.shape[2], self.a.shape[3]))

    def tensor(self):
        if self._t is None:
            self._t = concat_channels(self.a, self.b)
        return self._t


def concat_channels_deferred(a, b):
    if (VIRTUAL_CAT and SPLIT_DGRAD and FUSED_BLOCK and a.is_cuda and a.shape[1] == b.shape[1]
            and a.shape[1] % 16 == 0 and a.shape[0] == b.shape[0] and a.shape[2:] == b.shape[2:]):
        return CatParts(a, b)
    return concat_channels(a, b)


def basic_block_cat_fusable(parts, w1, ws):
    n, ca, h, w = parts.a.shape
    ci, co = 2 * ca, w1.shape[0]
    return (ws is not None and w1.shape[1] == ci and co % 4 == 0
            and H.call("smsut_conv2d_mfma_cat_supported", n, h, w, ci, co)
            and H.call("smsut_conv1x1_supported", ci, co) and H.call("smsut_conv1x1_tiles", n, h * w, co) > 0
            and H.call("smsut_conv2d_wgrad_mfma_supported", 3, 1, 1, ci, co))


def basic_block_cat(parts, w1, g1, b1, w2, g2, b2, ws, gs, bs, slope):
    return BasicBlockFn.apply(None, w1, g1, b1, w2, g2, b2, ws, gs, bs, slope, cl(parts.a), cl(parts.b))


BLOCK_POOL = bool(int(_os.environ.get("SMSUT_BLOCK_POOL", "1")))


def basic_block_pool_fusable(x, w1, ws):
    return (BLOCK_POOL and ws is not None and basic_block_fusable(x, w1, ws) and w1.shape[0] % 4 == 0
            and x.shape[2] % 2 == 0 and x.shape[3] % 2 == 0 and torch.is_grad_enabled() and (x.requires_grad or w1.requires_grad)
            and getattr(x, "_smsut_cat_parts", None) is None)


def basic_block_pool(x, w1, g1, b1, w2, g2, b2, ws, gs, bs, slope):
    return BasicBlockFn.apply(cl(x), w1, g1, b1, w2, g2, b2, ws, gs, bs, slope, None, None, True)


def basic_block(x, w1, g1, b1, w2, g2, b2, ws, gs, bs, slope):
    parts = getattr(x, "_smsut_cat_parts", None)
    if parts is not None and SPLIT_DGRAD and ws is not None and torch.is_grad_enabled():
        return BasicBlockFn.apply(cl(x).detach(), w1, g1, b1, w2, g2, b2, ws, gs, bs, slope, parts[0], parts[1])
    return BasicBlockFn.apply(cl(x), w1, g1, b1, w2, g2, b2, ws, gs, bs, slope)


class AddActFn(Function):

    @staticmethod
    def forward(ctx, a, b, slope):
        a = nhwc(a)
        if b is not None:
            b = nhwc(b)
            assert a.shape == b.shape
        y = new_act(*a.shape, a)
        H.call("smsut_add_act", a, b, y, a.numel(), float(slope), _s())
        ctx.save_for_backward(y)
        ctx.slope = float(slope)
        ctx.has_b = b is not None
        return y

    @staticmethod
    def backward(ctx, gy):
        (y,) = ctx.saved_tensors
        g = ActBwdFn.apply(gy, y, ctx.slope)
        return g, (g if ctx.has_b else None), None


class ActBwdFn(Function):
# ... 1395 lines not shown
```

### smsut-medicalimgsegmentation_amd/profiling.py

```python
from __future__ import annotations

import collections
from typing import Callable, Dict, List, Tuple

import torch

from . import _hip as H


def _k2(ints, i):
    return ints[i] * ints[i]


_CONV_FLOPS: Dict[str, Tuple[Callable[[List[int]], float], str]] = {
    "smsut_conv2d_fwd_generic": (lambda a: 2.0 * a[0] * a[4] * a[5] * a[3] * a[6] * a[7] * a[8], "direct"),
    "smsut_conv2d_dgrad_generic": (lambda a: 2.0 * a[0] * a[4] * a[5] * a[3] * a[6] * a[7] * a[8], "direct"),
    "smsut_conv2d_wgrad_generic": (lambda a: 2.0 * a[0] * a[4] * a[5] * a[3] * a[6] * a[7] * a[8], "direct"),
    "smsut_conv2d_fwd_mfma": (lambda a: 2.0 * a[0] * a[1] * a[2] * a[3] * a[4] * _k2(a, 5), "mfma"),
    "smsut_conv2d_wgrad_pair": (lambda a: 2.0 * (a[0] + a[1]) * a[3] * a[4] * a[5] * a[6] * 9, "mfma"),
    "smsut_conv2d_wgrad_pair_slabs": (lambda a: 2.0 * (a[0] + a[1]) * a[2] * a[3] * a[4] * a[5] * 9, "mfma"),
    "smsut_conv2d_fwd_mfma_stats": (lambda a: 2.0 * a[0] * a[1] * a[2] * a[3] * a[4] * _k2(a, 5), "mfma"),
    "smsut_conv2d_dgrad_mfma_bwdstats": (lambda a: 2.0 * a[0] * a[1] * a[2] * a[3] * a[4] * 9, "mfma"),
    "smsut_conv2d_wgrad_mfma": (lambda a: 2.0 * a[0] * a[1] * a[2] * a[3] * a[4] * _k2(a, 5), "mfma"),
    "smsut_conv2d_fwd_mfma_stats_inaff": (lambda a: 2.0 * a[0] * a[1] * a[2] * a[3] * a[4] * 9, "mfma"),
# ... 106 lines not shown
    "smsut_conv2d_fwd_mfma_stats_inaff": lambda a: _cv(a[0], a[1], a[2], a[3], a[4]),
    "smsut_conv2d_fwd_mfma_stats_cat": lambda a: _cv(a[0], a[1], a[2], a[3], a[4]),
    "smsut_conv2d_fwd_mfma_split": lambda a: _cv(a[1], a[2], a[3], a[4], a[5]),
    "smsut_conv2d_fwd_mfma_stats_sc": lambda a: _cv(a[0], a[1], a[2], a[3], a[4], extra_out=a[4]),
    "smsut_conv2d_fwd_mfma_stats_sc_f16": lambda a: _cv(a[0], a[1], a[2], a[3], a[4], extra_out=a[4]),
    "smsut_conv2d_dgrad_mfma_sc": lambda a: _cv(a[1], a[2], a[3], 2 * a[4], a[5]),
    "smsut_conv2d_dgrad_mfma_sc_f16": lambda a: _cv(a[1], a[2], a[3], 2 * a[4], a[5]),
    "smsut_conv2d_wgrad_sc_f16": lambda a: _cv(a[1], a[2], a[3], a[4], 2 * a[5]),
    "smsut_conv2d_wgrad_mfma": lambda a: _cv(a[0], a[1], a[2], a[3], a[4]),
    "smsut_conv2d_wgrad_mfma_inaff": lambda a: _cv(a[0], a[1], a[2], a[3], a[4]),
    "smsut_conv2d_wgrad_mfma_cat": lambda a: _cv(a[1], a[2], a[3], a[4], a[5]),
    "smsut_conv2d_wgrad_mfma_sc": lambda a: _cv(a[1], a[2], a[3], a[4], 2 * a[5]),
    "smsut_conv1x1_fwd": lambda a: 4.0 * a[0] * a[1] * (a[2] + a[3]),
    "smsut_conv1x1_wgrad": lambda a: 4.0 * a[0] * a[1] * (a[2] + a[3]),
    "smsut_convT2x2_fwd_mfma": lambda a: 4.0 * a[0] * a[1] * a[2] * (a[3] + 4 * a[4]),
    "smsut_convT2x2_dgrad_mfma": lambda a: 4.0 * a[0] * a[1] * a[2] * (a[3] + 4 * a[4]),
    "smsut_convT2x2_wgrad_mfma": lambda a: 4.0 * a[0] * a[1] * a[2] * (a[3] + 4 * a[4]),
    "smsut_convT2x2_fwd_ps": lambda a: 4.0 * a[0] * a[1] * a[2] * (a[3] + 4 * a[4]),
    "smsut_convT2x2_wgrad_ps": lambda a: 4.0 * a[0] * a[1] * a[2] * (a[3] + 4 * a[4]),
    "smsut_restail_fwd": lambda a: 4.0 * a[0] * a[1] * a[2] * 3,
    "smsut_restail_bwd": lambda a: 4.0 * a[0] * a[1] * a[2] * 5,
    "smsut_in_apply_bwd": lambda a: 4.0 * a[0] * a[1] * a[2] * 3,
    "smsut_instnorm_fwd": lambda a: 4.0 * a[0] * a[1] * a[2] * 2,
    "smsut_instnorm_fwd_partials": lambda a: 4.0 * a[1] * a[2] * a[3] * 2,
    "smsut_instnorm_bwd": lambda a: 4.0 * a[0] * a[1] * a[2] * 3,
    "smsut_instnorm_bwd2": lambda a: 4.0 * a[0] * a[1] * a[2] * 5,
    "smsut_restail_fwd_pool": lambda a: a[0] * a[1] * a[2] * a[3] * ((2.0 * 2 if a[4] else 4.0 * 2) + 4.0 * 1.25 + 0.25),
    "smsut_restail_bwd_pool": lambda a: a[0] * a[1] * a[2] * a[3] * ((2.0 * 2 if a[4] else 4.0 * 2) + 4.0 * 3.25 + 0.25),
    "smsut_instnorm_pool_fwd_partials": lambda a: 4.0 * a[1] * a[2] * a[3] * a[4] * 1.25,
    "smsut_instnorm_pool_bwd": lambda a: 4.0 * a[0] * a[1] * a[2] * a[3] * 2.25,
    "smsut_maxpool2_fwd": lambda a: 4.0 * a[0] * a[1] * a[2] * a[3] * 1.25,
    "smsut_maxpool2_bwd": lambda a: 4.0 * a[0] * a[1] * a[2] * a[3] * 2.25,
    "smsut_maxpool2_bwd_add": lambda a: 4.0 * a[0] * a[1] * a[2] * a[3] * 3.25,
    "smsut_avgpool2_fwd": lambda a: 4.0 * a[0] * a[1] * a[2] * a[3] * 1.25,
    "smsut_avgpool2_bwd": lambda a: 4.0 * a[0] * a[1] * a[2] * a[3] * 1.25,
    "smsut_add_act": lambda a: 4.0 * a[0] * 3,
    "smsut_conv2d_fwd_mfma_stats_f16_hs": lambda a: a[0] * a[1] * a[2] * (4.0 * a[3] + 2.0 * a[4]),
    "smsut_conv2d_fwd_mfma_stats_sc_f16_hs": lambda a: a[0] * a[1] * a[2] * (4.0 * a[3] + 2.0 * 2 * a[4]),
    "smsut_conv2d_dgrad_mfma_bwdstats_f16_hs": lambda a: a[0] * a[1] * a[2] * (4.0 * a[3] + 4.0 * a[4] + 2.0 * a[4]),
    "smsut_restail_fwd_hs": lambda a: a[0] * a[1] * a[2] * (2.0 * 2 + 4.0),
    "smsut_restail_bwd_hs": lambda a: a[0] * a[1] * a[2] * (4.0 * 3 + 2.0 * 2),
    "smsut_in_apply_bwd_hs": lambda a: a[0] * a[1] * a[2] * (4.0 * 2 + 2.0),
    "smsut_instnorm_fwd_partials_hs": lambda a: a[1] * a[2] * a[3] * (2.0 + 4.0),
    "smsut_instnorm_fwd_partials_hs2": lambda a: a[1] * a[2] * a[3] * (2.0 + 2.0),
    "smsut_conv2d_fwd_mfma_stats_f16_hsx": lambda a: a[0] * a[1] * a[2] * (2.0 * a[3] + 2.0 * a[4]),
    "smsut_conv2d_wgrad_f16_xh": lambda a: a[0] * a[1] * a[2] * (2.0 * a[3] + 4.0 * a[4]),
    "smsut_conv2d_wgrad_f16_xh_inaff": lambda a: a[0] * a[1] * a[2] * (2.0 * a[3] + 4.0 * a[4]),
    "smsut_conv2d_fwd_mfma_stats_inaff_f16_hsx": lambda a: a[0] * a[1] * a[2] * (2.0 * a[3] + 2.0 * a[4]),
    "smsut_act_bwd": lambda a: 4.0 * a[0] * 3,
    "smsut_tanh_fwd": lambda a: 4.0 * a[0] * 2,
    "smsut_tanh_bwd": lambda a: 4.0 * a[0] * 3,
    "smsut_edt_sq": lambda a: a[0] * a[2] * a[3] * (8.0 + 4.0 * a[1] + 2.0 * a[1] / 8.0),
    "smsut_sdf_final": lambda a: a[0] * a[2] * a[3] * (8.0 + 4.0 * a[1] + 4.0 * a[1]),
    "smsut_dtc_loss_fwd": lambda a: 4.0 * a[2] * a[3] * (2 * a[0] + a[1]),
    "smsut_dtc_loss_bwd": lambda a: 4.0 * a[2] * a[3] * (4 * a[0] + a[1]),
}


def bytes_of(name: str, conv_args) -> float:
    if name == "smsut_conv2d_wgrad_pair":
        n, h, w, cin, cout, rows = _pair_dims(conv_args)
        return _cv(n, h, w, cin, cout * (2 if rows == 10 else 1))
    ent = _BYTES.get(_base(name))
    return float(ent(_ints(name, conv_args))) if ent else 0.0


def _byte_class(name: str) -> str:
    n = _base(name)
    if "conv" in n:
        return "convolutions"
    if "restail" in n:
        return "residual tails"
    if "instnorm" in n or "in_apply" in n:
        return "InstanceNorm"
    return "pooling / pointwise"


class Row(collections.namedtuple("Row", "name args calls us flops exec_flops abytes")):
    @property
    def total_us(self):
        return self.us * self.calls


_NO_REPLAY = {"smsut_sgd_momentum_multi"}


def record_step(step: Callable[[], object]):
    rec = []
    orig = H.call

    def spy(name, *args):
        if name not in H._NO_STATUS and name not in _NO_REPLAY:
            rec.append((name, [H.ptr(a) if isinstance(a, torch.Tensor) or a is None else a for a in args]))
        return orig(name, *args)
    H.call = spy
    try:
        step()
        torch.cuda.synchronize()
    finally:
        H.call = orig
    return rec



def replay(rec, reps: int = 8) -> List[Row]:
    lib = H.load()
    groups = collections.OrderedDict()
    for name, conv in rec:
        sig = H.SIGNATURES[name].replace(" ", "")
        key = (name, tuple(a for c, a in zip(sig, conv) if c in "ilfd"))
        groups.setdefault(key, []).append(conv)
    e0, e1 = torch.cuda.Event(enable_timing=True), torch.cuda.Event(enable_timing=True)
    st = torch.cuda.current_stream()
    rows = []
    for (name, shp), calls in groups.items():
        conv = list(calls[0])
        fn = getattr(lib, name)
        conv[-1] = st.cuda_stream
        for _ in range(2):
            fn(*conv)
        torch.cuda.synchronize()
        e0.record(st)
        for _ in range(reps):
            fn(*conv)
        e1.record(st)
        torch.cuda.synchronize()
        fl = conv_flops_of(name, calls[0])
        rows.append(Row(name, shp, len(calls), e0.elapsed_time(e1) / reps * 1e3, fl, fl * executed_factor(name, calls[0]),
                        bytes_of(name, calls[0])))
    return rows


def summarize(rows: List[Row], peak_tflops: float) -> dict:
    conv = [r for r in rows if r.flops > 0]
    mfma = [r for r in conv if _CONV_FLOPS[_base(r.name)][1] == "mfma"]
    t_all = sum(r.total_us for r in rows)
    t_conv = sum(r.total_us for r in conv)
    f_conv = sum(r.flops * r.calls for r in conv)
    x_conv = sum(r.exec_flops * r.calls for r in conv)
    t_mfma = sum(r.total_us for r in mfma)
    f_mfma = sum(r.flops * r.calls for r in mfma)
    x_mfma = sum(r.exec_flops * r.calls for r in mfma)
    fam = collections.OrderedDict()
    for r in conv:
        k = ("wgrad" if "wgrad" in r.name else "fwd/dgrad") + (" 1x1" if "1x1" in r.name else (" convT" if "convT" in r.name else ""))
        t, f, x = fam.get(k, (0.0, 0.0, 0.0))
        fam[k] = (t + r.total_us, f + r.flops * r.calls, x + r.exec_flops * r.calls)
    byc = collections.OrderedDict()
    for r in rows:
        if r.abytes > 0:
            k = _byte_class(r.name)
            t, b = byc.get(k, (0.0, 0.0))
            byc[k] = (t + r.total_us, b + r.abytes * r.calls)
    tf = lambda f, t: round(f / (t * 1e-6) / 1e12, 2) if t else None
    fr = lambda f, t: round(f / (t * 1e-6) / 1e12 / peak_tflops, 4) if t else None
    return {
        "kernel_ms_all": round(t_all / 1e3, 3), "kernel_ms_conv": round(t_conv / 1e3, 3),
        "conv_gflop": round(f_conv / 1e9, 2), "conv_gflop_mfma_executed": round(x_conv / 1e9, 2),
        "step_conv_tflops": tf(f_conv, t_conv), "step_conv_frac": fr(f_conv, t_conv),
        "step_conv_tflops_mfma_executed": tf(x_conv, t_conv), "step_conv_frac_mfma_executed": fr(x_conv, t_conv),
        "mfma_conv_frac_algorithmic": fr(f_mfma, t_mfma), "mfma_conv_frac_executed": fr(x_mfma, t_mfma),
        "conv_share_of_kernel_time": round(t_conv / t_all, 4) if t_all else None,
        "algorithmic_gbytes": round(sum(b for _, b in byc.values()) / 1e9, 3),
        "algorithmic_bytes_by_class": {k: {"gbytes": round(b / 1e9, 3), "ms": round(t / 1e3, 3), "gbs": round(b / (t * 1e-6) / 1e9, 1)}
                                       for k, (t, b) in byc.items()},
        "families": {k: {"ms": round(t / 1e3, 3), "algorithmic_tflops": round(f / (t * 1e-6) / 1e12, 1),
                         "mfma_executed_tflops": round(x / (t * 1e-6) / 1e12, 1)} for k, (t, f, x) in fam.items()},
# ... 28 lines not shown
```

### smsut-medicalimgsegmentation_amd/trainer/uganConsisTrainer.py

```python
import os
import random
import time

import torch

from .. import config as cfg
from .. import graphs, ops
from .baseTrainer import LoaderCycle, make_parser, run_main, sgd_step
from .uganShp0Trainer import UGANShp0Trainer

SCALARS = ("D_real", "D_fake", "D_cls", "D_gp", "G_fake", "G_rec", "G_cls", "G_seg", "G_semi", "G_nce")


class UGANConsisTrainer(UGANShp0Trainer):
    def __init__(self, phase, args=None):
        super().__init__(phase, args)
        self.lambda_semi = 10
        self.semi_start_iter = 1000
        self._semi_on = False
        self._graphs = {}
        self._alias = None
        self._d_alias = None
        self._use_d_alias = os.environ.get("SMSUT_D_ALIAS", "1") not in ("0", "")
        self._d_async = os.environ.get("SMSUT_D_ASYNC_ALLREDUCE", "0") not in ("0", "")
# ... 80 lines not shown
                out_hat, _ = torch.func.functional_call(self.D, self._d_alias, (x_hat,))
            else:
                out_hat, _ = self.D(x_hat)
            return self.gradient_penalty(out_hat, x_hat)

        if self._d_fork and self._d_alias is not None:
            cur = torch.cuda.current_stream()
            if self._fork is None:
                self._fork = torch.cuda.Stream()
            self._fork.wait_stream(cur)
            with torch.cuda.stream(self._fork):
                gp = xhat_pass()

            def join():
                cur.wait_stream(self._fork)
                return gp
        else:
            join = xhat_pass
        with ops.first_order_pass():
            out_src, out_cls = self.D(torch.cat([x_real, x_fake], 0))
        d_real = ops.mean_all(out_src[:b], -1.0)
        d_cls = ops.cross_entropy_rows(out_cls[:b], modal_org)
        d_fake = ops.mean_all(out_src[b:], 1.0)
        d_gp = join()
        d_loss = d_real + d_fake + self.lambda_cls * d_cls + self.lambda_gp * d_gp
        d_loss.backward()
        if self._d_alias is not None:
            main, extra = [], []
            for name, p in self.D.named_parameters():
                a = self._d_alias[name]
                if a.grad is not None:
                    if p.grad is None:
                        p.grad = a.grad
                    else:
                        main.append(p.grad); extra.append(a.grad)
            if main:
                torch._foreach_add_(main, extra)
        return torch.stack([t.detach().float() for t in (d_real, d_fake, d_cls, d_gp)])

    def _g2gen_phase(self, x_real, vec_to, ids, y_real=None):
        y_fake, x_fake, feat_x = self._g1
        cut = None
        if self._g_split:
            xd, td = x_fake.detach().requires_grad_(True), feat_x.detach().requires_grad_(True)
            feat_x, _ = self.net.netF([td], patch_ids=[ids])
            cut, x_fake = (xd, td), xd
        if self._seg_batch:
            b, bs = x_real.size(0), y_real.size(0)
            with ops.wino_prepared(self.net, forms="f"):
                y_all = self.net(torch.cat([x_real, x_fake], 0), branch="seg")
                with ops.pair_wgrads():
                    x_rec, feat_f, _, _ = torch.func.functional_call(self.net, self._alias, (x_fake, vec_to),
                                                                     {"sample_ids": [ids], "branch": "tsl"})
            y_seg, y_rec = ops.row_segments(y_all, 0, bs, b, 2 * b)
            self._g1 = (y_seg, self._g1[1], self._g1[2])
            st_seg = self._keep_stats(0, self.loss.stats(y_seg, y_real))
            y_fake = y_all[:b].detach()
            self._seg_real = y_fake
        else:
            with ops.wino_prepared(self.net, forms="f"), ops.pair_wgrads():
                y_rec, x_rec, feat_f, _ = torch.func.functional_call(self.net, self._alias, (x_fake, vec_to),
                                                                     {"sample_ids": [ids]})
        g_rec = ops.l1_mean(x_real, x_rec)
        g_nce = self.nce_loss(feat_x, feat_f)
        if self._semi_on:
            pseudo = ops.argmax_channels(y_fake)
            st = self._keep_stats(1, self.loss.stats(y_rec, pseudo))
        else:
            pseudo, st = None, torch.zeros(1, device=self.device)
        self._g2 = (y_rec, pseudo, g_rec, g_nce) + ((cut,) if cut is not None else ())
        if self._seg_batch:
            return self._sflat
        return st

    def _g2a_phase(self, y_real, st_seg, st_semi, lambda_semi):
        bs = y_real.size(0)
        y_fake = self._g1[0]
        y_rec, pseudo, g_rec, g_nce, _ = self._g2
        g_seg = self.loss.from_stats(y_fake if y_fake.size(0) == bs else y_fake[:bs], y_real, st_seg)
        if self._semi_on:
            g_semi = self.loss.from_stats(y_rec, pseudo, st_semi)
        else:
            g_semi = torch.zeros((), device=self.device)
        with ops.wino_prepared(self.net, forms="b"):
            (self.lambda_rec * g_rec + self.lambda_seg * g_seg + lambda_semi * g_semi + 1.0 * g_nce).backward()
        return torch.stack([t.detach().float() for t in (g_rec, g_seg, g_semi, g_nce)])

    def _g2a1_phase(self, st_semi, lambda_semi):
        y_rec, pseudo, g_rec, g_nce, _ = self._g2
        if self._seg_batch:
            with ops.wino_prepared(self.net, forms="b"):
                (self.lambda_rec * g_rec + 1.0 * g_nce).backward()
            return torch.stack([t.detach().float() for t in (g_rec, g_nce)])
        if self._semi_on:
            g_semi = self.loss.from_stats(y_rec, pseudo, st_semi)
        else:
            g_semi = torch.zeros((), device=self.device)
        with ops.wino_prepared(self.net, forms="b"):
            (self.lambda_rec * g_rec + lambda_semi * g_semi + 1.0 * g_nce).backward()
        return torch.stack([t.detach().float() for t in (g_rec, g_semi, g_nce)])

    def _g2a2_phase(self, y_real, st_seg, st_semi=None, lambda_semi=None):
        y_fake = self._g1[0]
        g_seg = self.loss.from_stats(y_fake if y_fake.size(0) == y_real.size(0) else y_fake[:y_real.size(0)], y_real, st_seg)
        if self._seg_batch:
            y_rec, pseudo = self._g2[0], self._g2[1]
            g_semi = self.loss.from_stats(y_rec, pseudo, st_semi) if self._semi_on else torch.zeros((), device=self.device)
            with ops.wino_prepared(self.net, forms="b"):
                (self.lambda_seg * g_seg + lambda_semi * g_semi).backward()
            return torch.stack([t.detach().float() for t in (g_seg, g_semi)])
        with ops.wino_prepared(self.net, forms="b"):
            (self.lambda_seg * g_seg).backward()
        return g_seg.detach().float().reshape(1)

    def _g2d_phase(self, modal_trg):
        xd2 = self._g1[1].detach().requires_grad_(True)
        with ops.wino_prepared(self.D):
            with ops.first_order_pass():
                out_src, out_cls = self.D(xd2)
            g_fake = ops.mean_all(out_src, -1.0)
            g_cls = ops.cross_entropy_rows(out_cls, modal_trg)
            (g_fake + self.lambda_cls * g_cls).backward()
        self._gx_d = xd2.grad
        return torch.stack([t.detach().float() for t in (g_fake, g_cls)])

    def _g2c_phase(self):
        _, x_fake, t_e5 = self._g1
        xd, td = self._g2[4]
        with ops.wino_prepared(self.net, forms="b"):
            torch.autograd.backward([x_fake, t_e5], [xd.grad + self._gx_d, td.grad])
            ops.pair_flush()
        self._g1 = self._g2 = self._gx_d = self._seg_real = None
        main, extra = [], []
        for name, p in self.net.named_parameters():
            a = self._alias[name]
            if a.grad is not None:
                if p.grad is None:
                    p.grad = a.grad
                else:
                    main.append(p.grad); extra.append(a.grad)
        if main:
            torch._foreach_add_(main, extra)
        return torch.zeros(1, device=self.device)

    def _g2_phase(self, y_real, modal_trg, st_seg, st_semi, lambda_semi):
        with ops.wino_prepared(self.net, forms="b"), ops.wino_prepared(self.D):
            return self._g2_phase_body(y_real, modal_trg, st_seg, st_semi, lambda_semi)

    def _g2_phase_body(self, y_real, modal_trg, st_seg, st_semi, lambda_semi):
        bs = y_real.size(0)
        y_fake, x_fake, _ = self._g1
        y_rec, pseudo, g_rec, g_nce = self._g2
        def d_pass():
            with ops.first_order_pass():
                out_src, out_cls = self.D(x_fake)
            return ops.mean_all(out_src, -1.0), ops.cross_entropy_rows(out_cls, modal_trg)

        fork = self._d_fork and self._g2_fork
        if fork:
            cur = torch.cuda.current_stream()
            if self._fork is None:
                self._fork = torch.cuda.Stream()
            self._fork.wait_stream(cur)
            with torch.cuda.stream(self._fork):
                g_fake, g_cls = d_pass()
        else:
            g_fake, g_cls = d_pass()
        g_seg = self.loss.from_stats(y_fake if y_fake.size(0) == bs else y_fake[:bs], y_real, st_seg)
        if self._semi_on:
            g_semi = self.loss.from_stats(y_rec, pseudo, st_semi)
        else:
            g_semi = torch.zeros((), device=self.device)
        if fork:
            cur.wait_stream(self._fork)
        g_loss = g_fake + self.lambda_rec * g_rec + self.lambda_cls * g_cls + self.lambda_seg * g_seg \
            + lambda_semi * g_semi + 1.0 * g_nce
        g_loss.backward()
        ops.pair_flush()
        self._g1 = self._g2 = None
        main, extra = [], []
        for name, p in self.net.named_parameters():
            a = self._alias[name]
            if a.grad is not None:
                if p.grad is None:
                    p.grad = a.grad
                else:
                    main.append(p.grad); extra.append(a.grad)
        if main:
            torch._foreach_add_(main, extra)
        return torch.stack([t.detach().float() for t in (g_fake, g_rec, g_cls, g_seg, g_semi, g_nce)])

    def _run_phase(self, name, fn, inputs, params, rebind=()):
        use_graph = graphs.graphs_enabled() and self._eager_done
        if not use_graph:
            if self._graphs:
                graphs.invalidate_grad_bindings()
            for p in params:
                p.grad = None
            return fn(*inputs)
        key = (name, self._semi_on, self._geom) + tuple(tuple(t.shape) for t in inputs)
        g = self._graphs.get(key)
        if g is None:
            g = self._graphs[key] = graphs.GraphedPhase(fn, inputs, params, warmup=0, rebind_params=rebind)
            return g.static_out
        return g(*inputs)

    def graph_report(self):
        captured = sorted({k[0] for k in self._graphs if isinstance(k, tuple)})
        whole = set(captured) in ({"D", "G1", "G2", "G2gen"}, {"D", "G1", "G2a", "G2c", "G2d", "G2gen"},
                                  {"D", "G1", "G2a1", "G2a2", "G2c", "G2d", "G2gen"})
        mode = "graph" if whole else ("eager" if not captured else "graph(" + ",".join(captured) + ")")
        return {"mode": mode, "captured": captured, "fallback": False,
                "policy": os.environ.get("SMSUT_GRAPH", "default")}

    def train_iteration(self, x_real, y_real, modal_org, mj=None, alpha=None, sample_ids=None):
        lambda_semi = self.lambda_semi * self.sigmoid_rampup(self.epoch, cfg.max_epoch)
        self._geom = (tuple(x_real.shape), tuple(y_real.shape))
        ops.pair_reset()
        if mj is None:
            mj = random.randint(0, cfg.n_modal - 1)
        modal_org = self._to_device_async(modal_org)
        modal_trg = torch.full_like(modal_org, mj)
        vec_org = torch.zeros(modal_org.numel(), cfg.n_modal, device=self.device).scatter_(1, modal_org[:, None], 1.0)
        vec_trg = torch.zeros_like(vec_org)
        vec_trg[:, mj] = 1.0
        vec_ot, vec_to = vec_trg - vec_org, vec_org - vec_trg
        if alpha is None:
            alpha = torch.randn(x_real.size(0), 1, 1, 1, device=self.device)
        if sample_ids is None:
            hw = (x_real.shape[2] // 16) * (x_real.shape[3] // 16)
            torch.randperm(hw, device=self.device)
            ids = torch.randperm(hw, device=self.device)[: min(64, hw)]
        else:
            ids = sample_ids[0].to(self.device)
        self._semi_on = self.iter >= self.semi_start_iter
        lam_t = self._lambda_semi_t.fill_(lambda_semi)
        if self._alias is None:
            self._alias = {k: p.detach().requires_grad_(True) for k, p in self.net.named_parameters()}
        if self._use_d_alias and self._d_alias is None:
            self._d_alias = {k: p.detach().requires_grad_(True) for k, p in self.D.named_parameters()}
        g_params = list(self.net.parameters())
        d_params = list(self.D.parameters()) + (list(self._d_alias.values()) if self._d_alias else [])

        x_fake, st_seg = self._run_phase("G1", self._g1_phase, (x_real, vec_ot, ids, y_real), [])
        if self._probe:
            self._finite_probe("G1", [("x_fake", x_fake)])

        cur = torch.cuda.current_stream()
        overlap = self._d_overlap
        side_c = self._d_side_compute and not overlap
        if overlap or side_c:
            if self._side is None:
                self._side = torch.cuda.Stream()
            self._side.wait_stream(cur)
        d_work = None
        with torch.cuda.stream(self._side if (overlap or side_c) else cur):
            d_scal = self._run_phase("D", self._d_phase, (x_real, x_fake, modal_org, alpha), d_params)
            if self._probe:
                self._finite_probe("D", [("d_scalars", d_scal)] + [("grad " + k, p.grad) for k, p in self.D.named_parameters()])
            if not side_c:
                d_work = self.d_reducer.begin()
# ... 147 lines not shown
```

Before: 823.1.

## Defer weight-gradient split reductions and batch them into one multi-job kernel

Weight-gradient kernels that write split-K partial slabs no longer launch their own reduction kernel right away. Inside a finish_wgrads context they record a job, and the deferred jobs are later run by a single wgrad_finish_multi launch that looks up each block's job with a binary search. That launch can also accumulate into existing gradients. The goal is fewer small reduction launches and less per-launch overhead during backward, at the cost of host-side job planning, workspace buffers that must stay alive until the flush, and more complex gradient-parking logic.

```diff
diff --git a/include/smsut_hip.h b/include/smsut_hip.h
--- a/include/smsut_hip.h
+++ b/include/smsut_hip.h
@@ -115,6 +115,14 @@
                                   int NA, const float* xB, const float* gyB, const float* meanB ,
                                   const float* rstdB , int NB, const float* gamma , const float* beta ,
                                   float slope, float* workspace, int H, int W, int Cin, int Cout, void* stream);
+int smsut_slab_sum_splits(const float* part, float* out, int wsize, int splits, void* stream);
+int smsut_slab_sum_parts(const float* part, float* out, int wsize, int splits, void* stream);
+int smsut_slab_reduce_chunks(const float* part, float* out, int wsize, int chunks, void* stream);
+int smsut_wgrad_defer_begin(void);
+int smsut_wgrad_defer_take(void* jobs_host, int cap);
+int smsut_wgrad_finish_job_bytes(void);
+int smsut_wgrad_finish_plan(void* jobs_host, int njobs);
+int smsut_wgrad_finish_multi(const void* jobs, int njobs, int nblocks, void* stream);
 int smsut_conv1x1_fwd_cat(const float* xa, const float* xb, int ca, const float* w, float* y, float* stats ,
                           int N, int HW, int Kdim, int Ndim, void* stream);
 int smsut_conv1x1_wgrad_cat(const float* xa, const float* xb, int ca, const float* gy, float* gw, float* workspace, int N,
diff --git a/smsut-medicalimgsegmentation_amd/csrc/conv1x1.hip b/smsut-medicalimgsegmentation_amd/csrc/conv1x1.hip
--- a/smsut-medicalimgsegmentation_amd/csrc/conv1x1.hip
+++ b/smsut-medicalimgsegmentation_amd/csrc/conv1x1.hip
@@ -1,4 +1,5 @@
 #include "common.h"
+#include "slab_sum.h"
 
 namespace {
 
@@ -221,32 +222,7 @@
 __global__ void __launch_bounds__(TPB)
 sum_parts(const float* __restrict__ part, float* __restrict__ out, int wsize, int splits) {
   __shared__ float4 sm[TPB];
-  const int col = threadIdx.x & 15, sl = threadIdx.x >> 4;
-  const int e = (blockIdx.x * 16 + col) * 4;
-  float4 t0 = make_float4(0.f, 0.f, 0.f, 0.f), t1 = t0, t2 = t0, t3 = t0;
-  if (e < wsize) {
-    int c = sl;
-    for (; c + 48 < splits; c += 64) {
-      const float4 v0 = *(const float4*)(part + (size_t)c * wsize + e);
-      const float4 v1 = *(const float4*)(part + (size_t)(c + 16) * wsize + e);
-      const float4 v2 = *(const float4*)(part + (size_t)(c + 32) * wsize + e);
-      const float4 v3 = *(const float4*)(part + (size_t)(c + 48) * wsize + e);
-      t0.x += v0.x; t0.y += v0.y; t0.z += v0.z; t0.w += v0.w; t1.x += v1.x; t1.y += v1.y; t1.z += v1.z; t1.w += v1.w;
-      t2.x += v2.x; t2.y += v2.y; t2.z += v2.z; t2.w += v2.w; t3.x += v3.x; t3.y += v3.y; t3.z += v3.z; t3.w += v3.w;
-    }
-    for (; c < splits; c += 16) {
-      const float4 v = *(const float4*)(part + (size_t)c * wsize + e);
-      t0.x += v.x; t0.y += v.y; t0.z += v.z; t0.w += v.w;
-    }
-  }
-  sm[threadIdx.x] = make_float4((t0.x + t1.x) + (t2.x + t3.x), (t0.y + t1.y) + (t2.y + t3.y), (t0.z + t1.z) + (t2.z + t3.z),
-                                (t0.w + t1.w) + (t2.w + t3.w));
-  __syncthreads();
-  if (sl == 0 && e < wsize) {
-    float4 t = sm[col];
-    for (int l = 1; l < 16; ++l) { const float4 v = sm[l * 16 + col]; t.x += v.x; t.y += v.y; t.z += v.z; t.w += v.w; }
-    *(float4*)(out + e) = t;
-  }
+  sum_splits_body<16, false>(part, out, wsize, splits, blockIdx.x, sm);
 }
 
 struct Plan1 { int splits; int64_t pps; };
@@ -457,7 +433,15 @@
   if (cit == 2) conv1x1_wgrad<2, 2, true><<<grid, TPB, 0, st>>>(x, gy, workspace, P, Cin, Nd, p.pps, nullptr, 0, W);
   else conv1x1_wgrad<1, 2, true><<<grid, TPB, 0, st>>>(x, gy, workspace, P, Cin, Nd, p.pps, nullptr, 0, W);
   const int wsize = Cin * Nd;
-  sum_parts<<<(wsize + 63) / 64, TPB, 0, st>>>(workspace, gw, wsize, p.splits);
+  if (!smsut_finish_defer(workspace, gw, wsize, p.splits, SMSUT_FINISH_SUM_PARTS))
+    sum_parts<<<(wsize + 63) / 64, TPB, 0, st>>>(workspace, gw, wsize, p.splits);
+  SMSUT_LAUNCH_CHECK();
+  return SMSUT_OK;
+}
+
+int smsut_slab_sum_parts(const float* part, float* out, int wsize, int splits, void* stream) {
+  SMSUT_REQUIRE(part && out && wsize > 0 && wsize % 4 == 0 && splits > 0);
+  sum_parts<<<(wsize + 63) / 64, TPB, 0, (hipStream_t)stream>>>(part, out, wsize, splits);
   SMSUT_LAUNCH_CHECK();
   return SMSUT_OK;
 }
@@ -482,7 +466,8 @@
   else if (cot == 2) conv1x1_wgrad<1, 2><<<grid, TPB, 0, st>>>(x, gy, workspace, P, Cin, Cout, p.pps, x2, ca);
   else conv1x1_wgrad<1, 1><<<grid, TPB, 0, st>>>(x, gy, workspace, P, Cin, Cout, p.pps, x2, ca);
   const int wsize = Cin * Cout;
-  sum_parts<<<(wsize + 63) / 64, TPB, 0, st>>>(workspace, gw, wsize, p.splits);
+  if (!smsut_finish_defer(workspace, gw, wsize, p.splits, SMSUT_FINISH_SUM_PARTS))
+    sum_parts<<<(wsize + 63) / 64, TPB, 0, st>>>(workspace, gw, wsize, p.splits);
   SMSUT_LAUNCH_CHECK();
   return SMSUT_OK;
 }
diff --git a/smsut-medicalimgsegmentation_amd/csrc/conv_mfma_wgrad.hip b/smsut-medicalimgsegmentation_amd/csrc/conv_mfma_wgrad.hip
--- a/smsut-medicalimgsegmentation_amd/csrc/conv_mfma_wgrad.hip
+++ b/smsut-medicalimgsegmentation_amd/csrc/conv_mfma_wgrad.hip
@@ -1,5 +1,6 @@
 #include "conv_mfma.h"
 #include "conv_wgrad_rr.h"
+#include "slab_sum.h"
 
 namespace {
 
@@ -652,47 +653,54 @@
 template <int COLS>
 __global__ void __launch_bounds__(TPB)
 sum_splits(const float* __restrict__ part, float* __restrict__ out, int wsize, int splits) {
-  constexpr int LANES = TPB / COLS;
   __shared__ float4 sm[TPB];
-  const int col = threadIdx.x % COLS, sl = threadIdx.x / COLS;
-  const int e = (blockIdx.x * COLS + col) * 4;
-  float4 t0 = make_float4(0.f, 0.f, 0.f, 0.f), t1 = t0, t2 = t0, t3 = t0;
-  if (e < wsize) {
-    const float* p = part + e;
-    int c = sl;
-    for (; c + 3 * LANES < splits; c += 4 * LANES) {
-      const float4 v0 = *(const float4*)(p + (size_t)c * wsize);
-      const float4 v1 = *(const float4*)(p + (size_t)(c + LANES) * wsize);
-      const float4 v2 = *(const float4*)(p + (size_t)(c + 2 * LANES) * wsize);
-      const float4 v3 = *(const float4*)(p + (size_t)(c + 3 * LANES) * wsize);
-      t0.x += v0.x; t0.y += v0.y; t0.z += v0.z; t0.w += v0.w;
-      t1.x += v1.x; t1.y += v1.y; t1.z += v1.z; t1.w += v1.w;
-      t2.x += v2.x; t2.y += v2.y; t2.z += v2.z; t2.w += v2.w;
-      t3.x += v3.x; t3.y += v3.y; t3.z += v3.z; t3.w += v3.w;
-    }
-    for (; c < splits; c += LANES) {
-      const float4 v = *(const float4*)(p + (size_t)c * wsize);
-      t0.x += v.x; t0.y += v.y; t0.z += v.z; t0.w += v.w;
-    }
-  }
-  sm[threadIdx.x] = make_float4((t0.x + t1.x) + (t2.x + t3.x), (t0.y + t1.y) + (t2.y + t3.y),
-                                (t0.z + t1.z) + (t2.z + t3.z), (t0.w + t1.w) + (t2.w + t3.w));
-  __syncthreads();
-  if (sl == 0 && e < wsize) {
-    float4 t = sm[col];
-    for (int l = 1; l < LANES; ++l) {
-      const float4 v = sm[l * COLS + col];
-      t.x += v.x; t.y += v.y; t.z += v.z; t.w += v.w;
-    }
-    *(float4*)(out + e) = t;
-  }
+  sum_splits_body<COLS, false>(part, out, wsize, splits, blockIdx.x, sm);
 }
 
 inline void launch_sum_splits(const float* part, float* out, int wsize, int splits, hipStream_t st) {
-  if (wsize >= 32768) sum_splits<64><<<(wsize + 255) / 256, TPB, 0, st>>>(part, out, wsize, splits);
-  else if (wsize >= 8192) sum_splits<32><<<(wsize + 127) / 128, TPB, 0, st>>>(part, out, wsize, splits);
+  if (smsut_finish_defer(part, out, wsize, splits, SMSUT_FINISH_SUM_SPLITS)) return;
+  const int cols = sum_splits_cols(wsize);
+  if (cols == 64) sum_splits<64><<<(wsize + 255) / 256, TPB, 0, st>>>(part, out, wsize, splits);
+  else if (cols == 32) sum_splits<32><<<(wsize + 127) / 128, TPB, 0, st>>>(part, out, wsize, splits);
   else sum_splits<16><<<(wsize + 63) / 64, TPB, 0, st>>>(part, out, wsize, splits);
 }
+
+inline int finish_job_blocks(const SmsutFinishJob& j) {
+  const int per = j.kind == SMSUT_FINISH_SUM_SPLITS ? 4 * sum_splits_cols(j.wsize) : 64;
+  return (j.wsize + per - 1) / per;
+}
+__global__ void __launch_bounds__(TPB)
+wgrad_finish_multi(const SmsutFinishJob* __restrict__ jobs, int njobs) {
+  __shared__ float4 sm[TPB];
+  int lo = 0, hi = njobs - 1;
+  while (lo < hi) {
+    const int mid = (lo + hi + 1) >> 1;
+    if (jobs[mid].blk0 <= (int)blockIdx.x) lo = mid; else hi = mid - 1;
+  }
+  const SmsutFinishJob j = jobs[lo];
+  const int blk = blockIdx.x - j.blk0;
+  if (j.kind == SMSUT_FINISH_REDUCE_CHUNKS) {
+    if (j.accumulate) reduce_chunks_body<true>(j.part, j.out, j.wsize, j.splits, blk, (double*)sm);
+    else reduce_chunks_body<false>(j.part, j.out, j.wsize, j.splits, blk, (double*)sm);
+    return;
+  }
+  const int cols = j.kind == SMSUT_FINISH_SUM_PARTS ? 16 : sum_splits_cols(j.wsize);
+  if (cols == 64) {
+    if (j.accumulate) sum_splits_body<64, true>(j.part, j.out, j.wsize, j.splits, blk, sm);
+    else sum_splits_body<64, false>(j.part, j.out, j.wsize, j.splits, blk, sm);
+  } else if (cols == 32) {
+    if (j.accumulate) sum_splits_body<32, true>(j.part, j.out, j.wsize, j.splits, blk, sm);
+    else sum_splits_body<32, false>(j.part, j.out, j.wsize, j.splits, blk, sm);
+  } else {
+    if (j.accumulate) sum_splits_body<16, true>(j.part, j.out, j.wsize, j.splits, blk, sm);
+    else sum_splits_body<16, false>(j.part, j.out, j.wsize, j.splits, blk, sm);
+  }
+}
+
+constexpr int DEFER_CAP = 4;
+thread_local bool t_defer_on = false;
+thread_local int t_defer_n = 0;
+thread_local SmsutFinishJob t_defer[DEFER_CAP];
 
 constexpr int PW_UNR = 8;
 __global__ void __launch_bounds__(TPB)
@@ -1085,7 +1093,58 @@
 
 }
 
+bool smsut_finish_defer(const float* part, float* out, int wsize, int splits, int kind) {
+  if (!t_defer_on) return false;
+  if (t_defer_n < DEFER_CAP) t_defer[t_defer_n] = SmsutFinishJob{part, out, wsize, splits, kind, 0, 0, 0};
+  ++t_defer_n;
+  return true;
+}
+
 extern "C" {
+
+int smsut_wgrad_defer_begin(void) {
+  t_defer_on = true;
+  t_defer_n = 0;
+  return SMSUT_OK;
+}
+int smsut_wgrad_defer_take(void* jobs_host, int cap) {
+  const int n = t_defer_n;
+  t_defer_on = false;
+  t_defer_n = 0;
+  if (n > DEFER_CAP || n > cap || (n && !jobs_host)) return SMSUT_EINVAL;
+  for (int i = 0; i < n; ++i) ((SmsutFinishJob*)jobs_host)[i] = t_defer[i];
+  return n;
+}
+int smsut_slab_sum_splits(const float* part, float* out, int wsize, int splits, void* stream) {
+  SMSUT_REQUIRE(part && out && wsize > 0 && wsize % 4 == 0 && splits > 0);
+  launch_sum_splits(part, out, wsize, splits, (hipStream_t)stream);
+  SMSUT_LAUNCH_CHECK();
+  return SMSUT_OK;
+}
+int smsut_wgrad_finish_job_bytes(void) { return (int)sizeof(SmsutFinishJob); }
+int smsut_wgrad_finish_plan(void* jobs_host, int njobs) {
+  SMSUT_REQUIRE(njobs >= 0 && (jobs_host || njobs == 0));
+  SmsutFinishJob* j = (SmsutFinishJob*)jobs_host;
+  int64_t blocks = 0;
+  for (int i = 0; i < njobs; ++i) {
+    SMSUT_REQUIRE(j[i].part && j[i].out && j[i].wsize > 0 && j[i].splits > 0 && (j[i].accumulate == 0 || j[i].accumulate == 1));
+    SMSUT_REQUIRE(j[i].kind == SMSUT_FINISH_SUM_SPLITS || j[i].kind == SMSUT_FINISH_SUM_PARTS || j[i].kind == SMSUT_FINISH_REDUCE_CHUNKS);
+    SMSUT_REQUIRE(j[i].kind == SMSUT_FINISH_REDUCE_CHUNKS || (j[i].wsize % 4 == 0 && ((uintptr_t)j[i].part | (uintptr_t)j[i].out) % 16 == 0));
+    j[i].blk0 = (int)blocks;
+    j[i].reserved = 0;
+    blocks += finish_job_blocks(j[i]);
+    SMSUT_REQUIRE(blocks < (1ll << 30));
+  }
+  return (int)blocks;
+}
+int smsut_wgrad_finish_multi(const void* jobs, int njobs, int nblocks, void* stream) {
+  SMSUT_REQUIRE(njobs >= 0 && nblocks >= 0 && (njobs == 0) == (nblocks == 0));
+  if (njobs == 0) return SMSUT_OK;
+  SMSUT_REQUIRE(jobs && nblocks >= njobs);
+  wgrad_finish_multi<<<nblocks, TPB, 0, (hipStream_t)stream>>>((const SmsutFinishJob*)jobs, njobs);
+  SMSUT_LAUNCH_CHECK();
+  return SMSUT_OK;
+}
 
 #ifdef SMSUT_STAMPS
 int smsut_dbg_wgrad_stamps(void* buf, int base) {
diff --git a/smsut-medicalimgsegmentation_amd/csrc/conv_naive.hip b/smsut-medicalimgsegmentation_amd/csrc/conv_naive.hip
--- a/smsut-medicalimgsegmentation_amd/csrc/conv_naive.hip
+++ b/smsut-medicalimgsegmentation_amd/csrc/conv_naive.hip
@@ -1,4 +1,5 @@
 #include "common.h"
+#include "slab_sum.h"
 
 namespace {
 
@@ -117,24 +118,7 @@
 __global__ void __launch_bounds__(TPB)
 reduce_chunks(const float* __restrict__ part, float* __restrict__ out, int wsize, int chunks) {
   __shared__ double sm[TPB];
-  const int e = blockIdx.x * 64 + (threadIdx.x & 63);
-  const int lane_c = threadIdx.x >> 6;
-  double s = 0.0;
-  if (e < wsize) {
-    int c = lane_c;
-    for (; c + 28 < chunks; c += 32) {
-      float v[8];
-#pragma unroll
-      for (int u = 0; u < 8; ++u) v[u] = part[(size_t)(c + 4 * u) * wsize + e];
-#pragma unroll
-      for (int u = 0; u < 8; ++u) s += (double)v[u];
-    }
-    for (; c < chunks; c += 4) s += (double)part[(size_t)c * wsize + e];
-  }
-  sm[threadIdx.x] = s;
-  __syncthreads();
-  if (lane_c == 0 && e < wsize)
-    out[e] = (float)(sm[threadIdx.x] + sm[threadIdx.x + 64] + sm[threadIdx.x + 128] + sm[threadIdx.x + 192]);
+  reduce_chunks_body<false>(part, out, wsize, chunks, blockIdx.x, sm);
 }
 
 __global__ void __launch_bounds__(TPB)
@@ -230,7 +214,15 @@
   const int chunks = (int)cdiv64(npix, ppc);
   hipStream_t st = (hipStream_t)stream;
   conv_wgrad_partial<<<dim3((wsize + TPB - 1) / TPB, chunks), TPB, 0, st>>>(x, gy, workspace, g, wsize, npix, ppc);
-  reduce_chunks<<<(wsize + 63) / 64, TPB, 0, st>>>(workspace, gw, wsize, chunks);
+  if (!smsut_finish_defer(workspace, gw, wsize, chunks, SMSUT_FINISH_REDUCE_CHUNKS))
+    reduce_chunks<<<(wsize + 63) / 64, TPB, 0, st>>>(workspace, gw, wsize, chunks);
+  SMSUT_LAUNCH_CHECK();
+  return SMSUT_OK;
+}
+
+int smsut_slab_reduce_chunks(const float* part, float* out, int wsize, int chunks, void* stream) {
+  SMSUT_REQUIRE(part && out && wsize > 0 && chunks > 0);
+  reduce_chunks<<<(wsize + 63) / 64, TPB, 0, (hipStream_t)stream>>>(part, out, wsize, chunks);
   SMSUT_LAUNCH_CHECK();
   return SMSUT_OK;
 }
@@ -248,9 +240,10 @@
   const int chunks = (int)cdiv64(rows, rpc);
   hipStream_t st = (hipStream_t)stream;
   colsum_partial<<<chunks, TPB, 0, st>>>(x, workspace, rows, C, (int)rpc);
-  reduce_chunks<<<(C + 63) / 64, TPB, 0, st>>>(workspace, out, C, chunks);
-  SMSUT_LAUNCH_CHECK();
-  return SMSUT_OK;
-}
-
-}
+  if (!smsut_finish_defer(workspace, out, C, chunks, SMSUT_FINISH_REDUCE_CHUNKS))
+    reduce_chunks<<<(C + 63) / 64, TPB, 0, st>>>(workspace, out, C, chunks);
+  SMSUT_LAUNCH_CHECK();
+  return SMSUT_OK;
+}
+
+}
diff --git a/smsut-medicalimgsegmentation_amd/csrc/slab_sum.h b/smsut-medicalimgsegmentation_amd/csrc/slab_sum.h
--- /dev/null
+++ b/smsut-medicalimgsegmentation_amd/csrc/slab_sum.h
@@ -0,0 +1,89 @@
+#pragma once
+#include "common.h"
+
+namespace {
+
+constexpr int SLAB_TPB = 256;
+
+template <int COLS, bool ACC>
+__device__ __forceinline__ void sum_splits_body(const float* __restrict__ part, float* __restrict__ out, int wsize, int splits, int blk,
+                                                float4* sm) {
+  constexpr int LANES = SLAB_TPB / COLS;
+  const int col = threadIdx.x % COLS, sl = threadIdx.x / COLS;
+  const int e = (blk * COLS + col) * 4;
+  float4 t0 = make_float4(0.f, 0.f, 0.f, 0.f), t1 = t0, t2 = t0, t3 = t0;
+  if (e < wsize) {
+    const float* p = part + e;
+    int c = sl;
+    for (; c + 3 * LANES < splits; c += 4 * LANES) {
+      const float4 v0 = *(const float4*)(p + (size_t)c * wsize);
+      const float4 v1 = *(const float4*)(p + (size_t)(c + LANES) * wsize);
+      const float4 v2 = *(const float4*)(p + (size_t)(c + 2 * LANES) * wsize);
+      const float4 v3 = *(const float4*)(p + (size_t)(c + 3 * LANES) * wsize);
+      t0.x += v0.x; t0.y += v0.y; t0.z += v0.z; t0.w += v0.w;
+      t1.x += v1.x; t1.y += v1.y; t1.z += v1.z; t1.w += v1.w;
+      t2.x += v2.x; t2.y += v2.y; t2.z += v2.z; t2.w += v2.w;
+      t3.x += v3.x; t3.y += v3.y; t3.z += v3.z; t3.w += v3.w;
+    }
+    for (; c < splits; c += LANES) {
+      const float4 v = *(const float4*)(p + (size_t)c * wsize);
+      t0.x += v.x; t0.y += v.y; t0.z += v.z; t0.w += v.w;
+    }
+  }
+  sm[threadIdx.x] = make_float4((t0.x + t1.x) + (t2.x + t3.x), (t0.y + t1.y) + (t2.y + t3.y),
+                                (t0.z + t1.z) + (t2.z + t3.z), (t0.w + t1.w) + (t2.w + t3.w));
+  __syncthreads();
+  if (sl == 0 && e < wsize) {
+    float4 t = sm[col];
+    for (int l = 1; l < LANES; ++l) {
+      const float4 v = sm[l * COLS + col];
+      t.x += v.x; t.y += v.y; t.z += v.z; t.w += v.w;
+    }
+    if constexpr (ACC) {
+      const float4 o = *(const float4*)(out + e);
+      t = make_float4(o.x + t.x, o.y + t.y, o.z + t.z, o.w + t.w);
+    }
+    *(float4*)(out + e) = t;
+  }
+}
+
+template <bool ACC>
+__device__ __forceinline__ void reduce_chunks_body(const float* __restrict__ part, float* __restrict__ out, int wsize, int chunks, int blk,
+                                                   double* sm) {
+  const int e = blk * 64 + (threadIdx.x & 63);
+  const int lane_c = threadIdx.x >> 6;
+  double s = 0.0;
+  if (e < wsize) {
+    int c = lane_c;
+    for (; c + 28 < chunks; c += 32) {
+      float v[8];
+#pragma unroll
+      for (int u = 0; u < 8; ++u) v[u] = part[(size_t)(c + 4 * u) * wsize + e];
+#pragma unroll
+      for (int u = 0; u < 8; ++u) s += (double)v[u];
+    }
+    for (; c < chunks; c += 4) s += (double)part[(size_t)c * wsize + e];
+  }
+  sm[threadIdx.x] = s;
+  __syncthreads();
+  if (lane_c == 0 && e < wsize) {
+    const float r = (float)(sm[threadIdx.x] + sm[threadIdx.x + 64] + sm[threadIdx.x + 128] + sm[threadIdx.x + 192]);
+    out[e] = ACC ? out[e] + r : r;
+  }
+}
+
+__host__ __device__ inline int sum_splits_cols(int wsize) { return wsize >= 32768 ? 64 : wsize >= 8192 ? 32 : 16; }
+
+}
+
+struct SmsutFinishJob {
+  const float* part;
+  float* out;
+  int wsize, splits;
+  int kind;
+  int accumulate;
+  int blk0;
+  int reserved;
+};
+enum { SMSUT_FINISH_SUM_SPLITS = 0, SMSUT_FINISH_SUM_PARTS = 1, SMSUT_FINISH_REDUCE_CHUNKS = 2 };
+bool smsut_finish_defer(const float* part, float* out, int wsize, int splits, int kind);
diff --git a/smsut-medicalimgsegmentation_amd/ops.py b/smsut-medicalimgsegmentation_amd/ops.py
--- a/smsut-medicalimgsegmentation_amd/ops.py
+++ b/smsut-medicalimgsegmentation_amd/ops.py
@@ -822,8 +822,11 @@
         return 0
     n = 0
     for key in list(_PAIR_STASH):
-        for mine, single, deliver in _PAIR_STASH.pop(key):
-            deliver(single(mine))
+        for mine, single, views in _PAIR_STASH.pop(key):
+            g = single(mine)
+            if g is not None:
+                for leaf, view in views(g):
+                    _add_grad(leaf, view)
             n += 1
     return n
 
@@ -843,27 +846,167 @@
         p.grad = p.grad + g
 
 
+WGRAD_FINISH = _os.environ.get("SMSUT_WGRAD_FINISH", "1") not in ("0", "")
+_FINISH = None
+_FINISH_KEEP = []
+_FINISH_MAX_JOBS = 256
+
+
+_JOB = "QQiiiiii"
+_FINISH_ARENA = [None, 0]
+
+
+def _finish_table(raw: bytes) -> torch.Tensor:
+    if not torch.cuda.is_current_stream_capturing():
+        t = torch.empty(len(raw), dtype=torch.uint8).pin_memory()
+    else:
+        if _FINISH_ARENA[0] is None or _FINISH_ARENA[1] + len(raw) > _FINISH_ARENA[0].numel():
+            raise RuntimeError("ops.finish_wgrads: no pinned table space left for a captured phase (run a phase eagerly first)")
+        t = _FINISH_ARENA[0][_FINISH_ARENA[1]:_FINISH_ARENA[1] + len(raw)]
+        _FINISH_ARENA[1] += (len(raw) + 63) // 64 * 64
+    t.copy_(torch.frombuffer(bytearray(raw), dtype=torch.uint8))
+    return t
+
+
+class _FinishScope:
+    def __init__(self):
+        import ctypes
+        import struct
+        self.struct = struct.Struct(_JOB)
+        self.jb = H.call("smsut_wgrad_finish_job_bytes")
+        assert self.jb == self.struct.size
+        self.buf = ctypes.create_string_buffer(_FINISH_MAX_JOBS * self.jb)
+        self.addr = ctypes.addressof(self.buf)
+        self.n = 0
+        self.keep = []
+        self.deliveries = []
+        self.launches = 0
+        if _FINISH_ARENA[0] is None and not torch.cuda.is_current_stream_capturing():
+            _FINISH_ARENA[0] = torch.empty(1 << 20, dtype=torch.uint8).pin_memory()
+
+    def call(self, name, *args):
+        if self.n + 4 > _FINISH_MAX_JOBS:
+            raise RuntimeError("ops.finish_wgrads: more than %d deferred reductions in one scope" % _FINISH_MAX_JOBS)
+        H.call("smsut_wgrad_defer_begin")
+        try:
+            H.call(name, *args)
+        finally:
+            got = H.call("smsut_wgrad_defer_take", self.addr + self.n * self.jb, 4)
+        if got < 0:
+            raise RuntimeError(f"ops.finish_wgrads: {name} recorded more reductions than a call may")
+        self.keep.extend(a for a in args if isinstance(a, torch.Tensor))
+        first, self.n = self.n, self.n + got
+        return first, got
+
+    def deliver(self, first, cnt, g, targets):
+        self.deliveries.append((first, cnt, g, targets))
+
+    def finish(self):
+        rounds, written, post = {}, {}, []
+        for first, cnt, g, targets in self.deliveries:
+            if cnt == 0:
+                for leaf, view in targets:
+                    _add_grad(leaf, view)
+                continue
+            assert cnt == 1, "one reduction per weight-gradient call"
+            base = g.data_ptr()
+            rec = list(self.struct.unpack_from(self.buf, first * self.jb))
+            assert rec[1] == base and rec[5] == 0, "ops.finish_wgrads: the record does not name the call's destination"
+            inplace = all(leaf.grad is not None for leaf, _ in targets)
+            if inplace:
+                d0 = targets[0][0].grad.data_ptr() - (targets[0][1].data_ptr() - base)
+                inplace = all(leaf.grad.dtype == torch.float32 and leaf.grad.stride() == view.stride() and leaf.grad.shape == view.shape
+                              and leaf.grad.data_ptr() - d0 == view.data_ptr() - base for leaf, view in targets)
+                inplace = inplace and sum(view.numel() for _, view in targets) == g.numel()
+            if inplace:
+                rec[1], rec[5] = d0, 1
+                self.struct.pack_into(self.buf, first * self.jb, *rec)
+                r, ow = written.get(d0, (-1, 0))
+                rounds[first], written[d0] = r + 1, (r + 1, ow)
+            else:
+                r, ow = written.get(base, (-1, 0))
+                rounds[first], written[base] = r + 1, (r + 1, ow + 1)
+                for leaf, view in targets:
+                    if leaf.grad is None:
+                        leaf.grad = view
+                    else:
+                        post.append((leaf, view))
+        assert all(ow <= 1 for _, ow in written.values()), "ops.finish_wgrads: a destination has two overwrite jobs"
+        assert len(rounds) == self.n, "ops.finish_wgrads: a recorded reduction was never handed to a leaf"
+        for r in range(max(rounds.values(), default=-1) + 1):
+            self._launch([i for i in range(self.n) if rounds[i] == r])
+        for leaf, view in post:
+            leaf.grad = leaf.grad + view
+
+    def _launch(self, idx):
+        jb = self.jb
+        raw = b"".join(self.buf.raw[i * jb:(i + 1) * jb] for i in idx)
+        planned = bytearray(raw)
+        import ctypes
+        cbuf = (ctypes.c_char * len(planned)).from_buffer(planned)
+        nblocks = H.call("smsut_wgrad_finish_plan", ctypes.addressof(cbuf), len(idx))
+        del cbuf
+        if nblocks <= 0:
+            raise RuntimeError("ops.finish_wgrads: the job table was refused")
+        host = _finish_table(bytes(planned))
+        dev = torch.empty(len(planned), dtype=torch.uint8, device=self.keep[0].device)
+        dev.copy_(host, non_blocking=True)
+        H.call("smsut_wgrad_finish_multi", dev, len(idx), nblocks, _s())
+        self.launches += 1
+        if torch.cuda.is_current_stream_capturing():
+            _FINISH_KEEP.append((host, dev))
+
+
+@contextlib.contextmanager
+def finish_wgrads():
+    global _FINISH
+    if _FINISH is not None or not WGRAD_FINISH:
+        yield
+        return
+    scope = _FINISH = _FinishScope()
+    try:
+        yield
+        _FINISH = None
+        scope.finish()
+    finally:
+        _FINISH = None
+
+
+def _deferrable(leaves) -> bool:
+    return _FINISH is not None and all(t is None or (t.is_leaf and t.requires_grad) for t in leaves)
+
+
+def _wgrad_to(views, g, name, *args):
+    targets = views(g) if _FINISH is not None else None
+    if targets is None or not _deferrable([leaf for leaf, _ in targets]):
+        H.call(name, *args)
+        return g
+    first, got = _FINISH.call(name, *args)
+    _FINISH.deliver(first, got, g, targets)
+    return None
+
+
 class WgradSet(NamedTuple):
     x: torch.Tensor; x2: Optional[torch.Tensor]; gy: torch.Tensor; gs: Optional[torch.Tensor]
     mean: Optional[torch.Tensor]; rstd: Optional[torch.Tensor]; n: int
 
 
-def _pair_wgrad(key, mine: WgradSet, launch, single, deliver):
+def _pair_wgrad(key, mine: WgradSet, launch, single, views):
     rows, ca, gamma, beta, slope, dims = launch
     lst = _PAIR_STASH.get(key)
     if not lst:
-        _PAIR_STASH.setdefault(key, []).append((mine, single, deliver))
+        _PAIR_STASH.setdefault(key, []).append((mine, single, views))
         return None
     other = lst.pop()[0]
     if not lst:
         del _PAIR_STASH[key]
     cat, aff, sc = int(mine.x2 is not None), int(mine.mean is not None), int(mine.gs is not None)
     if not H.call("smsut_conv2d_wgrad_pair_supported", mine.n, other.n, *dims, cat, aff, sc):
-        return single(mine) + single(other)
+        return single(mine, False) + single(other, False)
     gw = torch.empty(rows * dims[2] * dims[3], dtype=torch.float32, device=mine.x.device)
     ws = _ws(H.call("smsut_conv2d_wgrad_pair_ws", mine.n, other.n, *dims, cat, aff, sc), mine.x)
-    H.call("smsut_conv2d_wgrad_pair", *mine, *other, ca, gamma if aff else None, beta if aff else None, float(slope), gw, ws, *dims, _s())
-    return gw
+    return _wgrad_to(views, gw, "smsut_conv2d_wgrad_pair", *mine, *other, ca, gamma if aff else None, beta if aff else None, float(slope),
+                     gw, ws, *dims, _s())
 
 
 class BlockPlan(NamedTuple):
@@ -1070,7 +1213,7 @@
     return gy1, gg1, gb1, sc2
 
 
-def _bb_wgrad2(p: BlockPlan, b: BlockBwd, pair_w, y1, a1, gy2, w2, sc2, m1, r1, g1, b1, st):
+def _bb_wgrad2(p: BlockPlan, b: BlockBwd, leaves, y1, a1, gy2, w2, sc2, m1, r1, g1, b1, st):
     (n, h, w, _, co), slope = p[:5], p.slope
     if p.hs or b.f16w2:
         gw2 = new_weight(co, co, 3, 3, device=gy2.device)
@@ -1081,24 +1224,25 @@
             H.call("smsut_conv2d_wgrad_f16", a1, None, 0, gy2, gw2, wws, sc2, n, h, w, co, co, st)
         return gw2
 
-    def single2(t):
+    as_w2 = lambda g: torch.as_strided(g, (co, co, 3, 3), hwio_strides(co, co, 3, 3))
+    views2 = lambda g: [(leaves[1], as_w2(g))]
+
+    def single2(t, park=True):
         g = _vec(t.x, 9 * co * co)
         wws2 = _ws(H.call("smsut_conv2d_wgrad_mfma_ws", t.n, h, w, co, co, 3), t.x)
+        to = views2 if park else (lambda g: None)
         if t.mean is not None:
-            H.call("smsut_conv2d_wgrad_mfma_inaff", t.x, t.gy, g, wws2, t.mean, t.rstd, g1, b1, slope, t.n, h, w, co, co, _s())
-        else:
-            H.call("smsut_conv2d_wgrad_mfma", t.x, t.gy, g, wws2, t.n, h, w, co, co, 3, _s())
-        return g
-    as_w2 = lambda g: torch.as_strided(g, (co, co, 3, 3), hwio_strides(co, co, 3, 3))
+            return _wgrad_to(to, g, "smsut_conv2d_wgrad_mfma_inaff", t.x, t.gy, g, wws2, t.mean, t.rstd, g1, b1, slope, t.n, h, w, co, co, _s())
+        return _wgrad_to(to, g, "smsut_conv2d_wgrad_mfma", t.x, t.gy, g, wws2, t.n, h, w, co, co, 3, _s())
     mine2 = WgradSet(y1, None, gy2, None, m1, r1, n) if p.inaff else WgradSet(a1, None, gy2, None, None, None, n)
     if not b.pair2:
-        return as_w2(single2(mine2))
-    leaf2 = pair_w[1]
-    gw2 = _pair_wgrad(("w2", w2.data_ptr()), mine2, (9, 0, g1, b1, slope, (h, w, co, co)), single2, lambda g: _add_grad(leaf2, as_w2(g)))
+        gw2 = single2(mine2)
+    else:
+        gw2 = _pair_wgrad(("w2", w2.data_ptr()), mine2, (9, 0, g1, b1, slope, (h, w, co, co)), single2, views2)
     return None if gw2 is None else as_w2(gw2)
 
 
-def _bb_wgrad1(p: BlockPlan, b: BlockBwd, pair_w, x, x2, gy1, gs_t, w1, amax, st):
+def _bb_wgrad1(p: BlockPlan, b: BlockBwd, leaves, x, x2, gy1, gs_t, w1, amax, st):
     n, h, w, ci, co = p[:5]
     hw, ca = h * w, (p.cat[0] if p.virtual else 0)
     as_w1 = lambda g: torch.as_strided(g, (co, ci, 3, 3), hwio_strides(co, ci, 3, 3))
@@ -1115,35 +1259,36 @@
                sc1, n, h, w, ci, co, st)
         return as_w1(g10), as_ws(g10), sc1
     if b.fused_wsc:
-        def single1(t):
+        views1 = lambda g: [(leaves[0], as_w1(g)), (leaves[2], as_ws(g))]
+
+        def single1(t, park=True):
             g = _vec(t.x, 10 * ci * co)
-            H.call("smsut_conv2d_wgrad_mfma_sc", t.x, t.x2, ca, t.gy, t.gs, g,
-                   _ws(H.call("smsut_conv2d_wgrad_sc_ws", t.n, h, w, ci, co), t.x), t.n, h, w, ci, co, _s())
-            return g
+            return _wgrad_to(views1 if park else (lambda g: None), g, "smsut_conv2d_wgrad_mfma_sc", t.x, t.x2, ca, t.gy, t.gs, g,
+                             _ws(H.call("smsut_conv2d_wgrad_sc_ws", t.n, h, w, ci, co), t.x), t.n, h, w, ci, co, _s())
         mine1 = WgradSet(x, x2, gy1, gs_t, None, None, n)
         if b.pair1:
-            leaf1, leafs = pair_w[0], pair_w[2]
-            g10 = _pair_wgrad(("w1", w1.data_ptr()), mine1, (10, ca, None, None, p.slope, (h, w, ci, co)), single1,
-                              lambda g: (_add_grad(leaf1, as_w1(g)), _add_grad(leafs, as_ws(g))))
+            g10 = _pair_wgrad(("w1", w1.data_ptr()), mine1, (10, ca, None, None, p.slope, (h, w, ci, co)), single1, views1)
         else:
             g10 = single1(mine1)
         return (None, None, sc1) if g10 is None else (as_w1(g10), as_ws(g10), sc1)
     gw1 = new_weight(co, ci, 3, 3, device=x.device)
     wws = _ws(H.call("smsut_conv2d_wgrad_f16_ws", n, h, w, ci, co) if b.f16w1 else H.call("smsut_conv2d_wgrad_mfma_ws", n, h, w, ci, co, 3), x)
+    to1 = lambda g: [(leaves[0], g)]
     if b.f16w1:
         H.call("smsut_conv2d_wgrad_f16", x, x2, ca, gy1, gw1, wws, sc1, n, h, w, ci, co, st)
     elif p.virtual:
-        H.call("smsut_conv2d_wgrad_mfma_cat", x, x2, ca, gy1, gw1, wws, n, h, w, ci, co, 3, st)
+        gw1 = _wgrad_to(to1, gw1, "smsut_conv2d_wgrad_mfma_cat", x, x2, ca, gy1, gw1, wws, n, h, w, ci, co, 3, st)
     else:
-        H.call("smsut_conv2d_wgrad_mfma", x, gy1, gw1, wws, n, h, w, ci, co, 3, st)
+        gw1 = _wgrad_to(to1, gw1, "smsut_conv2d_wgrad_mfma", x, gy1, gw1, wws, n, h, w, ci, co, 3, st)
     if not p.has_sc:
         return gw1, None, sc1
     gws = new_weight(co, ci, 1, 1, device=x.device)
     wws1 = _ws(H.call("smsut_conv1x1_wgrad_ws", n, hw, ci, co), x)
+    tos = lambda g: [(leaves[2], g)]
     if p.virtual:
-        H.call("smsut_conv1x1_wgrad_cat", x, x2, ca, gs_t, gws, wws1, n, hw, ci, co, st)
+        gws = _wgrad_to(tos, gws, "smsut_conv1x1_wgrad_cat", x, x2, ca, gs_t, gws, wws1, n, hw, ci, co, st)
     else:
-        H.call("smsut_conv1x1_wgrad", x, gs_t, gws, wws1, n, hw, ci, co, st)
+        gws = _wgrad_to(tos, gws, "smsut_conv1x1_wgrad", x, gs_t, gws, wws1, n, hw, ci, co, st)
     return gw1, gws, sc1
 
 
@@ -1193,7 +1338,7 @@
         if p.has_sc and not p.fused_sc:
             s, ms, rs = _bb_shortcut(p, x, x2, ws, st)
         out, pooled, ctx.pool_idx = _bb_tail(p, y2, m2, r2, g2, b2, s if p.has_sc else x, ms, rs, gs, bs, st)
-        ctx.pair_w = leaves if p.pair else None
+        ctx.leaves = leaves
         ctx.set_materialize_grads(False)
         ctx.save_for_backward(x, x2, w1, w2, ws, y1, a1, y2, s, out, m1, r1, m2, r2, ms, rs, g1, b1, g2,
                               *((gs, b2, bs) if p.has_sc else (None, None, None)))
@@ -1216,8 +1361,8 @@
         gy2, gs_t, gg2, gb2, ggs, gbs, amax = _bb_tail_bwd(p, b, g_out, g_pooled, ctx.pool_idx, out, y2, m2, r2, g2, b2,
                                                            s if p.has_sc else x, ms, rs, gs, bs, st)
         gy1, gg1, gb1, sc2 = _bb_dgrad2(p, b, gy2, w2, y1, m1, r1, g1, b1, amax, st)
-        gw2 = _bb_wgrad2(p, b, ctx.pair_w, y1, a1, gy2, w2, sc2, m1, r1, g1, b1, st)
-        gw1, gws, sc1 = _bb_wgrad1(p, b, ctx.pair_w, x, x2, gy1, gs_t, w1, amax, st)
+        gw2 = _bb_wgrad2(p, b, ctx.leaves, y1, a1, gy2, w2, sc2, m1, r1, g1, b1, st)
+        gw1, gws, sc1 = _bb_wgrad1(p, b, ctx.leaves, x, x2, gy1, gs_t, w1, amax, st)
         gx, ga, gb = _bb_dgrad1(p, b, gy1, gs_t, w1, ws, sc1, st) if b.dx else (None, None, None)
         return gx, gw1, gg1, gb1, gw2, gg2, gb2, gws, ggs, gbs, None, ga, gb, None
 
diff --git a/smsut-medicalimgsegmentation_amd/profiling.py b/smsut-medicalimgsegmentation_amd/profiling.py
--- a/smsut-medicalimgsegmentation_amd/profiling.py
+++ b/smsut-medicalimgsegmentation_amd/profiling.py
@@ -212,7 +212,7 @@
         return self.us * self.calls
 
 
-_NO_REPLAY = {"smsut_sgd_momentum_multi"}
+_NO_REPLAY = {"smsut_sgd_momentum_multi", "smsut_wgrad_finish_multi"}
 
 
 def record_step(step: Callable[[], object]):
diff --git a/smsut-medicalimgsegmentation_amd/trainer/uganConsisTrainer.py b/smsut-medicalimgsegmentation_amd/trainer/uganConsisTrainer.py
--- a/smsut-medicalimgsegmentation_amd/trainer/uganConsisTrainer.py
+++ b/smsut-medicalimgsegmentation_amd/trainer/uganConsisTrainer.py
@@ -186,21 +186,21 @@
             g_semi = self.loss.from_stats(y_rec, pseudo, st_semi)
         else:
             g_semi = torch.zeros((), device=self.device)
-        with ops.wino_prepared(self.net, forms="b"):
+        with ops.wino_prepared(self.net, forms="b"), ops.finish_wgrads():
             (self.lambda_rec * g_rec + self.lambda_seg * g_seg + lambda_semi * g_semi + 1.0 * g_nce).backward()
         return torch.stack([t.detach().float() for t in (g_rec, g_seg, g_semi, g_nce)])
 
     def _g2a1_phase(self, st_semi, lambda_semi):
         y_rec, pseudo, g_rec, g_nce, _ = self._g2
         if self._seg_batch:
-            with ops.wino_prepared(self.net, forms="b"):
+            with ops.wino_prepared(self.net, forms="b"), ops.finish_wgrads():
                 (self.lambda_rec * g_rec + 1.0 * g_nce).backward()
             return torch.stack([t.detach().float() for t in (g_rec, g_nce)])
         if self._semi_on:
             g_semi = self.loss.from_stats(y_rec, pseudo, st_semi)
         else:
             g_semi = torch.zeros((), device=self.device)
-        with ops.wino_prepared(self.net, forms="b"):
+        with ops.wino_prepared(self.net, forms="b"), ops.finish_wgrads():
             (self.lambda_rec * g_rec + lambda_semi * g_semi + 1.0 * g_nce).backward()
         return torch.stack([t.detach().float() for t in (g_rec, g_semi, g_nce)])
 
@@ -210,10 +210,10 @@
         if self._seg_batch:
             y_rec, pseudo = self._g2[0], self._g2[1]
             g_semi = self.loss.from_stats(y_rec, pseudo, st_semi) if self._semi_on else torch.zeros((), device=self.device)
-            with ops.wino_prepared(self.net, forms="b"):
+            with ops.wino_prepared(self.net, forms="b"), ops.finish_wgrads():
                 (self.lambda_seg * g_seg + lambda_semi * g_semi).backward()
             return torch.stack([t.detach().float() for t in (g_seg, g_semi)])
-        with ops.wino_prepared(self.net, forms="b"):
+        with ops.wino_prepared(self.net, forms="b"), ops.finish_wgrads():
             (self.lambda_seg * g_seg).backward()
         return g_seg.detach().float().reshape(1)
 
@@ -231,7 +231,7 @@
     def _g2c_phase(self):
         _, x_fake, t_e5 = self._g1
         xd, td = self._g2[4]
-        with ops.wino_prepared(self.net, forms="b"):
+        with ops.wino_prepared(self.net, forms="b"), ops.finish_wgrads():
             torch.autograd.backward([x_fake, t_e5], [xd.grad + self._gx_d, td.grad])
             ops.pair_flush()
         self._g1 = self._g2 = self._gx_d = self._seg_real = None
@@ -279,8 +279,9 @@
             cur.wait_stream(self._fork)
         g_loss = g_fake + self.lambda_rec * g_rec + self.lambda_cls * g_cls + self.lambda_seg * g_seg \
             + lambda_semi * g_semi + 1.0 * g_nce
-        g_loss.backward()
-        ops.pair_flush()
+        with ops.finish_wgrads():
+            g_loss.backward()
+            ops.pair_flush()
         self._g1 = self._g2 = None
         main, extra = [], []
         for name, p in self.net.named_parameters():
```

Result: no change. 823.7 (median of 2 runs) (+0.1%).
